# NVlabs/intrinsic3d

Measured on AMD Instinct MI355X. Metric: Gauss-Newton iterations/s at the finest SDF level, higher is better.
Workload: dtype f32

## Files before the change

### intrinsic3d_amd/csrc/device/kernels.hpp

```cpp
#pragma once
#include "common.hpp"
#include "p2p_device.hpp"

namespace i3d {

struct HashTable { unsigned long long* keys; int* vals; unsigned int mask; };
void launch_sort_keys(hipStream_t st, int N, const int* keys_xyz , unsigned long long* sort_keys, int* iota);
void launch_permute_grid(hipStream_t st, int N, const int* perm, const int* keys_xyz, const double* sdf, const double* sdf_ref,
                         const double* alb, const float* w, const uint8_t* rgb,
                         int* cx, int* cy, int* cz, int* rank, double* sdf0, double* x_sdf, double* x_alb, float* f_sdf, float* f_alb,
                         float* weight, uchar4* color);
void launch_hash_build(hipStream_t st, int N, const int* cx, const int* cy, const int* cz, HashTable t);
void launch_nbr_build(hipStream_t st, int N, const int* cx, const int* cy, const int* cz, HashTable t, int* nbr);
void launch_classify(hipStream_t st, GridView g, OptParams p, int* active_flag);
void launch_compact(hipStream_t st, int N, const int* active_flag, const int* active_scan, const uint8_t* flags, int* aidx, int* alist, uint8_t* aflags);
void launch_partition_blocks(hipStream_t st, GridView g, int A, int* alist, uint8_t* aflags, int* aidx);
void launch_group_rows(hipStream_t st, int A, const uint8_t* nrows, int* gmax);
void launch_anbr(hipStream_t st, int N, int A, int Acap, const int* alist, const int* nbr, const int* aidx, int* anbr);
void launch_scatter_sh(hipStream_t st, int N, const int* rank, const double* sh_visit , float* sh );
void launch_gather_visit(hipStream_t st, int N, const int* rank, const double* x_sdf, const double* x_alb, double* out_sdf, double* out_alb);
void launch_update_fields(hipStream_t st, int N, const int* rank, const double* sdf_ref, const double* alb, const uint8_t* rgb,
                          double* x_sdf, double* x_alb, float* f_sdf, float* f_alb, uchar4* color);

void launch_observe(hipStream_t st, GridView g, RowView r, OptParams p, const FrameConst* frames, const unsigned* cull_mask = nullptr, bool prefilter = false);
constexpr int CULL_BLOCK = 8, CULL_MAX_LEVELS = 12;
struct CullPyramid { int levels, cells; int bw[CULL_MAX_LEVELS], bh[CULL_MAX_LEVELS], off[CULL_MAX_LEVELS]; };
CullPyramid cull_pyramid(int w, int h);
void launch_depth_blocks(hipStream_t st, const FrameConst* frames, int K, int w, int h, float2* out);
void launch_group_cull(hipStream_t st, GridView g, RowView r, OptParams p, const FrameConst* frames, const float2* dblocks, float4* bounds, unsigned* mask);

void launch_build(hipStream_t st, GridView g, RowView r, OptParams p, const FrameConst* frames, bool with_jacobian, double* cost_out , double* scratch,
                  const double* cam9 = nullptr, const LmState* lm = nullptr);
void launch_weight_sums(hipStream_t st, RowView r, GridView g, bool with_cost, double* sums13 , double* scratch);

enum PassMode { PASS_GRAD = 0, PASS_JTJP = 1, PASS_COLNORM = 2 };
struct Seg2 { size_t off0, off1; int n; };
struct PassBuffers {
    float* C;
    float* treg;
    double* shared;
    double* blocks;
    float* part; int part_stride;
};
struct GradColBuffers {
    float* Cg; float* Cc;
    float* tregg; float* tregc;
    float* part; int part_stride;
    int col_off;
    double* cost_partials; double* cost_out;
};
int  launch_eg_gradcol(hipStream_t st, GridView g, RowView r, OptParams p, GradColBuffers b);
int  launch_eg_pass(hipStream_t st, PassMode mode, GridView g, RowView r, OptParams p, const float* u , PassBuffers b, const PcgState* state);
void launch_sum_rows(hipStream_t st, PassMode mode, int K, const float* part, int nrows, int stride, double* shared, double* blocks);
void launch_gather(hipStream_t st, PassMode mode, RowView r, PassBuffers b, float* out );
int  launch_gather_tail(hipStream_t st, RowView r, PassBuffers b, float* out, const float* S, const float* D2, const float* v, double* dot_partials ,
                        bool dot_atomic, const PcgState* state);
void launch_reduce_partials(hipStream_t st, const double* partials, int nblk, int ncomp, double* dst, const PcgState* state, bool assign = false);
void launch_shared_finalize(hipStream_t st, size_t tail_off, int K, OptParams p, const double* shared, float* out , bool tail, const float* S, const float* D2,
                            const float* v, double* dot_out, const PcgState* state);

void launch_fill(hipStream_t st, int n, float* x, float v);
void launch_fill_d(hipStream_t st, int n, double* x, double v);
void launch_int_to_double(hipStream_t st, const int* src, double* dst);
void launch_mul(hipStream_t st, int n, const float* a, const float* b, float* out);
void launch_scale_from_colnorm(hipStream_t st, int n, const float* c, const float* freemask, float* S, float* cm);
void launch_dot(hipStream_t st, int n, const float* a, const float* b, double* out , double* scratch);
void launch_count_above2(hipStream_t st, Seg2 sg, const float* a, const float* m, float tol, double* out, double* scratch);
void launch_count_above(hipStream_t st, int n, const float* a, const float* m, float tol, double* out, double* scratch);
void launch_dot2(hipStream_t st, Seg2 sg, const float* a, const float* b, double* out , double* scratch);
void launch_mul2(hipStream_t st, Seg2 sg, const float* a, const float* b, float* out);
void launch_freemask(hipStream_t st, RowView r, OptParams p, float* mask );

void launch_pcg_init(hipStream_t st, PcgState* state, int fixed_iterations, int max_iterations, const LmState* lm = nullptr);
int  launch_pcg_step(hipStream_t st, int mode, Seg2 sg, const float* p, const float* q, float* x, float* r, const float* b, const float* D2, const float* Minv,
                     float* z, const float* S_for_inline_q, double* partials , PcgState* state);
void launch_pcg_tail_x(hipStream_t st, size_t tail_off, int K, const float* p, float* x, const PcgState* state);
void launch_pcg_tail_a(hipStream_t st, int mode, size_t tail_off, int K, const float* Minv_blocks, const float* p, const float* q, float* x, float* r, const float* b,
                       const float* D2, float* z, const double* partials, int nblk, PcgState* state,
                       double* shared_zero, int nzero, int* host_flags, int seq,
                       const P2PDev& pd);
int  launch_pcg_direction(hipStream_t st, Seg2 sg, size_t tail_off, int ntail, const float* z, float* p, const float* S, float* u, const float* D2,
                          double* d2_partials , const PcgState* state);
void launch_pcg_tail_b(hipStream_t st, size_t tail_off, int K, OptParams p, double* shared, const double* pq_slice, const double* pq_partials, int nblk,
                       const double* pq_partials2, int nblk2, bool rowwise,
                       float* q, const float* S, const float* D2, const float* v, PcgState* state, const P2PDev& pd);
struct TilePlan {
    unsigned* lnbr;
    float* eaw_sym;
    int* halo_idx; int* halo_cnt;
    int* iota; int* ext_e; int* ext_pos;
    float* qh;
    int* ext_off;
    int* overflow;
    int T, hmax;
    int tile_first, ntiles_own;
    const int* ghost_tiles; int n_ghost;
    int det;
    const unsigned short* hp_off;
    const unsigned short* hp_src;
    int pull;
};
inline int tile_plan_pull_cap(int hmax) { return 4 * hmax; }
inline int tile_plan_hmax_of(int T) { return T == 1024 ? 2048 : 1536; }
inline int tile_plan_tiles_of(int A, int T) { return (A + T - 1) / T; }
size_t tile_plan_temp_bytes(size_t nslots);
hipError_t launch_tile_plan(hipStream_t st, RowView r, TilePlan t, int hmax_limit , void* temp, size_t temp_bytes);
void launch_eaw_sym(hipStream_t st, RowView r, TilePlan t, const int* cflag );
int  launch_eg_tile(hipStream_t st, RowView r, OptParams p, const float* u, TilePlan t, double* shared, float* qacc, double* pq_partials ,
                    const PcgState* state, float* cam_partials = nullptr, int cam_stride = 0);
void launch_ext_offsets(hipStream_t st, int n, const int* ext_e, int A, int* ext_off);
void eg_tile_launch_shape(const TilePlan& t, int K, int& blocks, int& tiles_per_block);

struct LadVec;
int  eg_tile_mr_max_systems(int K);
int  launch_eg_tile_mr(hipStream_t st, RowView r, OptParams p, TilePlan t, int nsys, const int* sys, const float* u0, float* qacc0, float* qh0, double* pq0 , float* cam0, int cam_stride,
                       const PcgState* st0 , const LadVec& lv);
int  launch_eg_tile_mr_pair(hipStream_t st, RowView r, OptParams p, TilePlan t, int na, int nb, const int* sys, const float* u0, float* qacc0, float* qh0, double* pq0 , float* cam0,
                            int cam_stride, const PcgState* st0, const LadVec& lv);

struct ShardArgs {
    P2PDev pd; RimLists rim; int seq;
    int n_slice_partials;
    int n_rim_wg;
    const float* zb; float* pb; float* ub; const float* cmb; int chunk;
};
struct LadVec {
    size_t vec;
    size_t qh;
    size_t cam;
    size_t part;
    size_t mblk;
    size_t tail;
    int sysid[LADDER_MAX];
};
struct Step3Args {
    int nq; int chunk4;
    const float4* p; const float4* qacc; float4* x; float4* r; const float4* b; float4* z;
    const float4* cm; const LmState* lm;
    const int* ext_off; const int* ext_pos; const float2* qh; int e0;
    const double* pq_partials; int n_pq; const double* d2_partials; int n_d2;
    int n_slice_wg;
    int K; int fix_poses, fix_intr, fix_dist;
    const float* cam_partials; int n_cam; int cam_stride; const float* Mblk;
    const float* tp; float* tx; float* tr; const float* tb; const float* tD2; float* tz; const float* tS;
    double* step_partials;
    PcgState* cur;
    int sharded; ShardArgs sh;
    int lad_sys;
    const double* redop; int redop_stride;
};
void launch_pcg_init3(hipStream_t st, PcgState* st2 , int fixed_iterations, int max_iterations, const LmState* lm = nullptr);
int  launch_pcg_dir3(hipStream_t st, bool init, Seg2 sg, size_t tail_off, int ntail, const float* z, float* p, const float* S, float* u, const float* D2, const float* cm, const LmState* lm,
                     const double* step_partials, int n_step, double* d2_partials, const PcgState* prev, PcgState* next, int* host_flags, int seq,
                     const ShardArgs* sa = nullptr);
void launch_rim_u(hipStream_t st, const ShardArgs& sa, const PcgState* state);
int  pcg_step3_slice_wgs(int n_entries, int cap = 0);
int  pcg_step3_tail_wgs(int K);
int  launch_pcg_step3(hipStream_t st, int mode , Step3Args a);
void launch_halo_fold(hipStream_t st, RowView r, TilePlan t, float* qacc, const PcgState* state);
void launch_pcg_init_lad(hipStream_t st, PcgState* st2_all , int B, int fixed_iterations, int max_iterations, const LmState* lm);
int  launch_pcg_dir3_lad(hipStream_t st, bool init, int nsys, Seg2 sg, size_t tail_off, int ntail, const float* z0, float* p0, const float* S, float* u0, const float* tD2_0, const float* cm, const LmState* lm,
                         const double* step_partials0, int n_step, double* d2_partials0, PcgState* st2_0, int prev_parity, int* host_flags0, int seq, const LadVec& lv,
                         int n_slice_partials = 0, const double* red4_0 = nullptr );
int  launch_pcg_step3_lad(hipStream_t st, int mode, int nsys, Step3Args a, const LadVec& lv);
void launch_lad_reduce_step(hipStream_t st, int nsys, const double* step_partials0, int n_slice, double* red4_0, const LadVec& lv);
void launch_lad_reduce_op(hipStream_t st, int nsys, const float* cam_partials0, int n_cam, int cam_stride, int NS, const double* pq_partials0, int n_pq, const double* d2_partials0, int n_d2,
                          double* redop0, int redop_stride, const LadVec& lv);

void launch_need_mask(hipStream_t st, RowView r, int slice, unsigned long long* need );
void launch_halo_items(hipStream_t st, int A, int slice, int me, const unsigned long long* need, unsigned long long* items, int* count , int cap);
void launch_tile_flags(hipStream_t st, int A, int T, const int* cflag, int* tileflag );
size_t halo_sort_temp_bytes(int cap);
hipError_t launch_halo_sort(hipStream_t st, void* temp, size_t temp_bytes, const unsigned long long* in, unsigned long long* out, int n);

void launch_candidate(hipStream_t st, GridView g, RowView r, int K, float sign, const float* step, const float* S, const double* x_shared, double* xc_sdf, double* xc_alb,
                      double* xc_shared, double* norms2 , const float* mask, double* scratch, const LmState* lm = nullptr);
void launch_accept(hipStream_t st, GridView g, RowView r, const double* xc_sdf, const double* xc_alb, const LmState* lm = nullptr);
void launch_set_double(hipStream_t st, double* dst, double v);
void launch_lm_init(hipStream_t st, LmState* lm, const double* cost, const double* ngrad, const double* nfree, double radius0, LmRecord* rec, int seq);
void launch_lm_begin(hipStream_t st, LmState* lm, int K, int fix_poses, int fix_intr, int fix_dist, const double* cdiag, const double* tri, float* Mblk,
                     const float* tc, const float* tS, float* tD2, float* tMinv, LmRecord* rec, int seq);
void launch_lm_diag_dev(hipStream_t st, int n, const float* c, const float* S, const LmState* lm, float* D2, float* Minv);
void launch_cand_frames(hipStream_t st, int K, const double* xc, const FrameConst* base, FrameConst* out, const LmState* lm);
void launch_lm_decide(hipStream_t st, LmState* lm, const PcgState* ps, const double* norms2, const double* cand_cost, int attempt, int lm_steps, LmRecord* rec, int seq,
                      int lad_next = -1 , int debug_invalid = 0);
void launch_lm_begin_lad(hipStream_t st, LmState* lm, int B, int K, int fix_poses, int fix_intr, int fix_dist, const double* cdiag, const double* tri, float* Mblk, size_t mblk_stride,
                         const float* tc, const float* tS, float* tD2, size_t tail_stride, LmRecord* rec, int seq);
void launch_mark_compute(hipStream_t st, RowView r, int* flag);
void launch_compact_list(hipStream_t st, int A, const int* flag, const int* scan, int* list);

}
```

### intrinsic3d_amd/csrc/device/pcg_fused.hip

```cpp
#include "kernels.hpp"
#include "reduce_device.hpp"
#include <cstring>

namespace i3d {

constexpr int PF_THREADS = 512;
constexpr int PF_MAX_WG = 512;
constexpr int PF_POSES_PER_WG = 10;

template <int NC>
static __device__ inline void reduce_partials_all(const double* __restrict__ P, int nblk, double (&tot)[NC], double* sm ,
                                                  const double* __restrict__ P2 = nullptr, int nblk2 = 0 ) {
    double v[NC];
#pragma unroll
    for (int k = 0; k < NC; ++k) v[k] = 0.0;
    for (int i = threadIdx.x; i < nblk; i += PF_THREADS) {
#pragma unroll
        for (int k = 0; k < NC; ++k) v[k] += P[(size_t)i * NC + k];
    }
    for (int i = threadIdx.x; i < nblk2; i += PF_THREADS) {
#pragma unroll
        for (int k = 0; k < NC; ++k) v[k] += P2[(size_t)i * NC + k];
    }
#pragma unroll
    for (int k = 0; k < NC; ++k) for (int o = 32; o > 0; o >>= 1) v[k] += __shfl_down(v[k], o, 64);
    if ((threadIdx.x & 63) == 0) {
#pragma unroll
        for (int k = 0; k < NC; ++k) sm[k * 8 + (threadIdx.x >> 6)] = v[k];
    }
    __syncthreads();
#pragma unroll
    for (int k = 0; k < NC; ++k) { double t = 0.0; for (int w = 0; w < PF_THREADS / 64; ++w) t += sm[k * 8 + w]; tot[k] = t; }
    __syncthreads();
}

__global__ void k_pcg_init3(PcgState* st2, int fixed_iterations, int max_iterations, const LmState* lm) {
    const bool over = lm && lm->done;
    for (int b = 0; b < 2; ++b) {
        PcgState* st = st2 + b;
        for (int k = 0; k < 4; ++k) st->acc[k] = 0.0;
        st->rho = 0.0; st->last_rho = 1.0; st->pq = 0.0; st->alpha = 0.0; st->beta = 0.0; st->xbr = 0.0; st->xr = 0.0; st->d2xx = 0.0;
        st->Q0 = 0.0; st->Q1 = 0.0; st->it = 0; st->done = (fixed_iterations == 0 || over) ? 1 : 0; st->fixed_iterations = fixed_iterations; st->max_iterations = max_iterations;
    }
}
void launch_pcg_init3(hipStream_t st, PcgState* st2, int fixed_iterations, int max_iterations, const LmState* lm) { k_pcg_init3<<<1, 1, 0, st>>>(st2, fixed_iterations, max_iterations, lm); }

static __device__ inline void lm_from_colnorm(float cm, float inv_radius, float& s, float& d2, float& minv) { s = lm_scale(cm); lm_diag(cm, s, inv_radius, d2, minv); }

template <int SH>
static __device__ __forceinline__ void pcg_dir3_body(int init, int n4, int seg4, size_t tail_rel, int ntail, const float* __restrict__ z, float* __restrict__ p,
                                                        const float* __restrict__ S, float* __restrict__ u, const float* __restrict__ tD2 ,
                                                        const float* __restrict__ cm, const float inv_radius, const double* __restrict__ step_partials, int n_step, double* __restrict__ d2_partials,
                                                        const PcgState* __restrict__ prev, PcgState* __restrict__ next, int* host_flags, int seq, const ShardArgs& sa,
                                                        const double* __restrict__ red4 = nullptr ) {
    __shared__ double sm[4 * 8];
    __shared__ double smx[SH == 1 ? 4 * P2P_MAX_RANKS : 1];
    auto publish = [&](int done) { if (host_flags) { __hip_atomic_store(&host_flags[2 * (seq & 1) + 1], done, __ATOMIC_RELAXED, __HIP_MEMORY_SCOPE_SYSTEM);
                                                     __hip_atomic_store(&host_flags[2 * (seq & 1)], seq, __ATOMIC_RELEASE, __HIP_MEMORY_SCOPE_SYSTEM); } };
    const int n_rim = SH == 1 ? sa.n_rim_wg : 0, n_main = SH ? (int)gridDim.x - n_rim - 1 : (int)gridDim.x;
    const int lid = SH == 1 ? ((int)blockIdx.x < n_rim ? n_main + 1 + (int)blockIdx.x : (int)blockIdx.x - n_rim) : (int)blockIdx.x;
    const bool rim_wg = SH == 1 && lid > n_main, tail_wg = SH ? lid == n_main : lid == n_main - 1;
    const bool writer = lid == 0 && threadIdx.x == 0;
    const float4* z4 = reinterpret_cast<const float4*>(z); float4* p4 = reinterpret_cast<float4*>(p);
    const float4* C4 = reinterpret_cast<const float4*>(cm); float4* u4 = reinterpret_cast<float4*>(u);
    if (prev->done) { if (writer) { *next = *prev; publish(prev->done); } return; }
    double tot[4];
    if (!SH) reduce_partials_all<4>(step_partials, n_step, tot, sm);
    else if (SH == 2) {
        reduce_partials_all<4>(step_partials + 4 * (size_t)sa.n_slice_partials, n_step - sa.n_slice_partials, tot, sm);
#pragma unroll
        for (int k = 0; k < 4; ++k) tot[k] += red4[k];
    } else {
        const unsigned e32 = p2p_pass_epoch(seq, P2P_X_DIR);
        if (rim_wg) {
            const RimLists& rl = sa.rim;
            for (int j = (lid - n_main - 1) * PF_THREADS + threadIdx.x; j < rl.n_send; j += n_rim * PF_THREADS) {
                const int e = rl.send_idx[j], k = rl.send_peer[j];
                p2p_put_rim(sa.pd, 0, e32, k, j - rl.send_off[k], sa.zb[e], sa.zb[(size_t)sa.chunk + e]);
            }
        }
        {   double loc[4];
            reduce_partials_all<4>(step_partials, sa.n_slice_partials, loc, sm);
            if (lid == 0 && threadIdx.x < 4) p2p_put_double_all(sa.pd, 0, e32, threadIdx.x, threadIdx.x == 0 ? loc[0] : threadIdx.x == 1 ? loc[1] : threadIdx.x == 2 ? loc[2] : loc[3]); }
        double tl[4];
        reduce_partials_all<4>(step_partials + 4 * (size_t)sa.n_slice_partials, n_step - sa.n_slice_partials, tl, sm);
        p2p_sum_all<4>(sa.pd, 0, e32, tot, smx);
#pragma unroll
        for (int k = 0; k < 4; ++k) tot[k] += tl[k];
    }
    int it = prev->it, done = 0; bool stop = false;
    double Q0 = prev->Q0, Q1 = prev->Q1, xbr = prev->xbr, xr = prev->xr, d2xx = prev->d2xx;
    if (!init) {
        xbr = tot[1]; xr = tot[2]; d2xx = tot[3];
        it = it + 1;
        Q1 = -tot[1];
        if (prev->fixed_iterations >= 0) { Q0 = Q1; if (it >= prev->fixed_iterations) { done = 1; stop = true; } }
        else {
            const double zeta = (double)it * (Q1 - Q0) / Q1;
            if (zeta < 0.1) { done = 1; stop = true; }
            else { Q0 = Q1; if (it >= prev->max_iterations) { done = 1; stop = true; } }
        }
    }
    double rho = prev->rho, last_rho = prev->last_rho, beta = prev->beta;
    if (!stop) {
        const double rho_new = tot[0];
        if (rho_new == 0.0 || isinf(rho_new) || isnan(rho_new)) { done = 2; stop = true; }
        else {
            if (it > 0) { const double bt = rho_new / prev->rho; if (bt == 0.0 || isinf(bt) || isnan(bt)) { done = 2; stop = true; } else beta = bt; }
            else beta = 0.0;
            if (!stop) { last_rho = prev->rho; rho = rho_new; }
        }
    }
    if (writer) {
        PcgState s = *prev;
        s.rho = rho; s.last_rho = last_rho; s.beta = beta; s.xbr = xbr; s.xr = xr; s.d2xx = d2xx; s.Q0 = Q0; s.Q1 = Q1; s.it = it; s.done = done; s.pq = 0.0;
        *next = s;
        publish(done);
    }
    if (stop) return;
    const float betaf = (float)beta; const bool first = it == 0;
    if (rim_wg) {
        const RimLists& rl = sa.rim; const unsigned e32 = p2p_pass_epoch(seq, P2P_X_DIR);
        for (int j = (lid - n_main - 1) * PF_THREADS + threadIdx.x; j < rl.n_recv; j += n_rim * PF_THREADS) {
            const int e = rl.recv_idx[j], k = rl.recv_peer[j];
            float zs, za; p2p_get_rim(sa.pd, 0, e32, k, j - rl.recv_off[k], zs, za);
            const size_t ea = (size_t)sa.chunk + e;
            const float ps = first ? zs : zs + betaf * sa.pb[e], pa = first ? za : za + betaf * sa.pb[ea];
            sa.pb[e] = ps; sa.pb[ea] = pa;
            sa.ub[e] = lm_scale(sa.cmb[e]) * ps; sa.ub[ea] = lm_scale(sa.cmb[ea]) * pa;
        }
        return;
    }
    double d2 = 0.0;
    if (!SH || !tail_wg) {
        for (int j = lid * PF_THREADS + threadIdx.x; j < 2 * n4; j += n_main * PF_THREADS) {
            const int i = j < n4 ? j : j - n4 + seg4;
            float4 pi = z4[i]; const float4 cv = C4[i];
            if (!first) { const float4 po = p4[i]; pi.x += betaf * po.x; pi.y += betaf * po.y; pi.z += betaf * po.z; pi.w += betaf * po.w; }
            p4[i] = pi;
            float4 sv, dd; float mi;
            lm_from_colnorm(cv.x, inv_radius, sv.x, dd.x, mi); lm_from_colnorm(cv.y, inv_radius, sv.y, dd.y, mi);
            lm_from_colnorm(cv.z, inv_radius, sv.z, dd.z, mi); lm_from_colnorm(cv.w, inv_radius, sv.w, dd.w, mi);
            u4[i] = make_float4(sv.x * pi.x, sv.y * pi.y, sv.z * pi.z, sv.w * pi.w);
            d2 += (double)dd.x * (double)pi.x * (double)pi.x + (double)dd.y * (double)pi.y * (double)pi.y + (double)dd.z * (double)pi.z * (double)pi.z + (double)dd.w * (double)pi.w * (double)pi.w;
        }
    }
    if (tail_wg) {
        for (int t = threadIdx.x; t < ntail; t += PF_THREADS) {
            const size_t i = tail_rel + t;
            const float pi = first ? z[i] : z[i] + betaf * p[i]; p[i] = pi; u[i] = S[i] * pi;
            d2 += (double)tD2[t] * (double)pi * (double)pi;
        }
    }
    { const double t = block_sum_d(d2); if (threadIdx.x == 0) d2_partials[lid] = t; }
}
template <int SH>
__global__ void __launch_bounds__(PF_THREADS, SH ? 4 : 1) k_pcg_dir3(int init, int n4, int seg4, size_t tail_rel, int ntail, const float* __restrict__ z, float* __restrict__ p,
                                                        const float* __restrict__ S, float* __restrict__ u, const float* __restrict__ D2 ,
                                                        const float* __restrict__ cm, const LmState* __restrict__ lm, const double* __restrict__ step_partials, int n_step, double* __restrict__ d2_partials,
                                                        const PcgState* __restrict__ prev, PcgState* __restrict__ next, int* host_flags, int seq, ShardArgs sa) {
    pcg_dir3_body<SH>(init, n4, seg4, tail_rel, ntail, z, p, S, u, D2 + tail_rel, cm, lm->inv_radius , step_partials, n_step, d2_partials, prev, next, host_flags, seq, sa);
}
template <bool COLL>
__global__ void __launch_bounds__(PF_THREADS, 1) k_pcg_dir3_lad(int init, int n4, int seg4, size_t tail_rel, int ntail, const float* __restrict__ z0, float* __restrict__ p0,
                                                        const float* __restrict__ S, float* __restrict__ u0, const float* __restrict__ tD2_0, const float* __restrict__ cm, const LmState* __restrict__ lm,
                                                        const double* __restrict__ step_partials0, int n_step, double* __restrict__ d2_partials0, PcgState* __restrict__ st2_0 , int prev_parity,
                                                        int* host_flags0, int seq, LadVec lv, int n_slice_partials, const double* __restrict__ red4_0) {
    const int j = lv.sysid[blockIdx.y];
    ShardArgs none; none.n_rim_wg = 0; none.n_slice_partials = n_slice_partials;
    const size_t vo = (size_t)j * lv.vec;
    pcg_dir3_body<COLL ? 2 : 0>(init, n4, seg4, tail_rel, ntail, z0 + vo, p0 + vo, S, u0 + vo, tD2_0 + (size_t)j * lv.tail, cm, lm->lad_inv_radius[j], step_partials0 + (size_t)j * lv.part, n_step,
                                d2_partials0 + (size_t)j * lv.part, st2_0 + 2 * j + prev_parity, st2_0 + 2 * j + (prev_parity ^ 1), host_flags0 + 4 * j, seq, none, COLL ? red4_0 + 4 * j : nullptr);
}

static int dir3_main_wgs(int n_entries, int cap) { int b = (n_entries / 2 + PF_THREADS - 1) / PF_THREADS; b = b < 1 ? 1 : b; return b > cap ? cap : b; }
int launch_pcg_dir3(hipStream_t st, bool init, Seg2 sg, size_t tail_off, int ntail, const float* z, float* p, const float* S, float* u, const float* D2, const float* cm, const LmState* lm,
                    const double* step_partials, int n_step, double* d2_partials, const PcgState* prev, PcgState* next, int* host_flags, int seq, const ShardArgs* sa) {
    const int n4 = sg.n >> 2, seg4 = (int)((sg.off1 - sg.off0) >> 2);
    const size_t o = sg.off0;
    if (!sa) {
        const int blocks = dir3_main_wgs(sg.n, PF_MAX_WG);
        ShardArgs none; std::memset(&none, 0, sizeof(none));
        k_pcg_dir3<0><<<blocks, PF_THREADS, 0, st>>>(init ? 1 : 0, n4, seg4, tail_off - o, ntail, z + o, p + o, S + o, u + o, D2 + o, cm + o, lm, step_partials, n_step, d2_partials, prev, next, host_flags, seq, none);
        return blocks;
    }
    const int cap = sa->pd.wg_cap > 0 ? sa->pd.wg_cap : PF_MAX_WG;
    const int n_main = dir3_main_wgs(sg.n, cap);
    k_pcg_dir3<1><<<sa->n_rim_wg + n_main + 1, PF_THREADS, 0, st>>>(init ? 1 : 0, n4, seg4, tail_off - o, ntail, z + o, p + o, S + o, u + o, D2 + o, cm + o, lm, step_partials, n_step, d2_partials, prev, next,
                                                                       host_flags, seq, *sa);
    return n_main;
}

int launch_pcg_dir3_lad(hipStream_t st, bool init, int nsys, Seg2 sg, size_t tail_off, int ntail, const float* z0, float* p0, const float* S, float* u0, const float* tD2_0, const float* cm, const LmState* lm,
                        const double* step_partials0, int n_step, double* d2_partials0, PcgState* st2_0, int prev_parity, int* host_flags0, int seq, const LadVec& lv,
                        int n_slice_partials, const double* red4_0) {
    const int n4 = sg.n >> 2, seg4 = (int)((sg.off1 - sg.off0) >> 2);
    const size_t o = sg.off0;
    const int blocks = dir3_main_wgs(sg.n, PF_MAX_WG);
    if (red4_0)
        k_pcg_dir3_lad<true><<<dim3(blocks + 1, nsys), PF_THREADS, 0, st>>>(init ? 1 : 0, n4, seg4, tail_off - o, ntail, z0 + o, p0 + o, S + o, u0 + o, tD2_0, cm + o, lm, step_partials0, n_step, d2_partials0,
                                                                            st2_0, prev_parity, host_flags0, seq, lv, n_slice_partials, red4_0);
    else
        k_pcg_dir3_lad<false><<<dim3(blocks, nsys), PF_THREADS, 0, st>>>(init ? 1 : 0, n4, seg4, tail_off - o, ntail, z0 + o, p0 + o, S + o, u0 + o, tD2_0, cm + o, lm, step_partials0, n_step, d2_partials0,
                                                                         st2_0, prev_parity, host_flags0, seq, lv, 0, nullptr);
    return blocks;
}

__global__ void __launch_bounds__(PF_THREADS) k_rim_u(ShardArgs sa, const PcgState* __restrict__ state) {
    if (state->done) return;
    const RimLists& rl = sa.rim; const unsigned e32 = p2p_pass_epoch(sa.seq, P2P_X_RESET_RIM);
    for (int j = blockIdx.x * PF_THREADS + threadIdx.x; j < rl.n_send; j += gridDim.x * PF_THREADS) {
        const int e = rl.send_idx[j], k = rl.send_peer[j];
        p2p_put_rim(sa.pd, 0, e32, k, j - rl.send_off[k], sa.ub[e], sa.ub[(size_t)sa.chunk + e]);
    }
    for (int j = blockIdx.x * PF_THREADS + threadIdx.x; j < rl.n_recv; j += gridDim.x * PF_THREADS) {
        const int e = rl.recv_idx[j], k = rl.recv_peer[j];
        float us, ua; p2p_get_rim(sa.pd, 0, e32, k, j - rl.recv_off[k], us, ua);
        sa.ub[e] = us; sa.ub[(size_t)sa.chunk + e] = ua;
    }
}
void launch_rim_u(hipStream_t st, const ShardArgs& sa, const PcgState* state) { if (sa.rim.n_send > 0 || sa.rim.n_recv > 0) k_rim_u<<<sa.n_rim_wg > 0 ? sa.n_rim_wg : 1, PF_THREADS, 0, st>>>(sa, state); }

enum { S3_INIT = 0, S3_NORMAL = 1, S3_XONLY = 2, S3_RESET = 3 };


struct S3Off { size_t v4, vo, qh2, part, cam, mblk, tail; int st, sys; };
struct S3In { float4 as, aa; int4 o; int o4; float4 x[2], p[2], b[2], cm[2], r[2]; };
template <int MODE> static __device__ inline void s3_load(const Step3Args& a, const S3Off& o, int q, S3In& v) {
    const float4* const qacc = a.qacc + o.v4; const float4* const x = a.x + o.v4; const float4* const p = a.p + o.v4; const float4* const r = a.r + o.v4;
    if (MODE == S3_NORMAL || MODE == S3_RESET) {
        v.as = qacc[q]; v.aa = qacc[q + a.chunk4];
        const int e = a.e0 + 4 * q;
        v.o = *reinterpret_cast<const int4*>(a.ext_off + e);
        v.o4 = a.ext_off[e + 4];
    }
#pragma unroll
    for (int seg = 0; seg < 2; ++seg) {
        const int i = q + seg * a.chunk4;
        v.cm[seg] = a.cm[i];
        if (MODE == S3_INIT) v.r[seg] = r[i];
        else {
            v.x[seg] = x[i];
            if (MODE != S3_RESET) v.p[seg] = p[i];
            if (MODE != S3_XONLY) { v.b[seg] = a.b[i]; if (MODE == S3_NORMAL) v.r[seg] = r[i]; }
        }
    }
}

template <int MODE, int SH>
static __device__ __forceinline__ void pcg_step3_body(const Step3Args& a, const S3Off& o) {
    __shared__ double sm[4 * 8];
    __shared__ double smx[SH == 1 ? P2P_MAX_RANKS : 1];
    __shared__ double camv[64];
    __shared__ double camred[8][64];
    __shared__ float rs[64];
    PcgState* const cur = a.cur + o.st;
    float4* const X = a.x + o.v4; float4* const R = a.r + o.v4; float4* const Z = a.z + o.v4;
    const double* const pq_partials = a.pq_partials + o.part; const double* const d2_partials = a.d2_partials + o.part; double* const step_partials = a.step_partials + o.part;
    const float2* const qh = a.qh + o.qh2; const float* const cam_partials = a.cam_partials + o.cam; const float* const Mblk = a.Mblk + o.mblk;
    const float* const tp = a.tp + o.vo; float* const tx = a.tx + o.vo; float* const tr = a.tr + o.vo; float* const tz = a.tz + o.vo; const float* const tD2 = a.tD2 + o.tail;
    const bool slice_wg = (int)blockIdx.x < a.n_slice_wg;
    const int q0 = blockIdx.x * PF_THREADS + threadIdx.x, qstride = a.n_slice_wg * PF_THREADS;
    S3In in;
    __shared__ int done_s;
    if (threadIdx.x == 0) done_s = cur->done;
    __syncthreads();
    if (done_s) return;
    const float inv_radius = o.sys >= 0 ? a.lm->lad_inv_radius[o.sys] : a.lm->inv_radius;
    float alpha = 0.0f;
    if (MODE == S3_NORMAL || MODE == S3_XONLY) {
        double t1[1];
        if (SH == 2) t1[0] = a.redop[(size_t)(o.sys < 0 ? 0 : o.sys) * a.redop_stride + 6 * a.K + 9] + d2_partials[a.n_d2];
        else reduce_partials_all<1>(pq_partials, a.n_pq, t1, sm, d2_partials, a.n_d2);
        if (SH == 1) {
            const unsigned e32 = p2p_pass_epoch(a.sh.seq, P2P_X_STEP);
            if (blockIdx.x == 0 && threadIdx.x == 0) p2p_put_double_all(a.sh.pd, 1, e32, 0, t1[0]);
            p2p_sum_all<1>(a.sh.pd, 1, e32, t1, smx);
            t1[0] += d2_partials[a.n_d2];
        }
        const double pq = t1[0];
        const double al = cur->rho / pq;
        const bool bad = !(pq > 0.0) || isinf(pq) || isinf(al);
        if (blockIdx.x == 0 && threadIdx.x == 0) { cur->pq = pq; if (bad) cur->done = 2; else cur->alpha = al; }
        if (bad) return;
        alpha = (float)al;
    }
    double s0 = 0.0, s1 = 0.0, s2 = 0.0, s3 = 0.0;
    if (slice_wg) {
        for (int q = q0; q < a.nq; q += qstride) {
            s3_load<MODE>(a, o, q, in);
            float accv[2][4];
            if (MODE == S3_NORMAL || MODE == S3_RESET) {
                const float4 as = in.as, aa = in.aa;
                accv[0][0] = as.x; accv[0][1] = as.y; accv[0][2] = as.z; accv[0][3] = as.w; accv[1][0] = aa.x; accv[1][1] = aa.y; accv[1][2] = aa.z; accv[1][3] = aa.w;
                const int ob[5] = {in.o.x, in.o.y, in.o.z, in.o.w, in.o4};
                for (int j0 = ob[0]; j0 < ob[4]; j0 += 8) {
                    int pos[8]; float2 hv[8];
#pragma unroll
                    for (int u = 0; u < 8; ++u) pos[u] = (j0 + u < ob[4]) ? a.ext_pos[j0 + u] : -1;
#pragma unroll
                    for (int u = 0; u < 8; ++u) hv[u] = pos[u] >= 0 ? qh[pos[u]] : make_float2(0.0f, 0.0f);
#pragma unroll
                    for (int u = 0; u < 8; ++u) {
                        const int j = j0 + u;
                        if (j < ob[4]) {
#pragma unroll
                            for (int k = 0; k < 4; ++k) { const bool mine = j >= ob[k] && j < ob[k + 1]; accv[0][k] += mine ? hv[u].x : 0.0f; accv[1][k] += mine ? hv[u].y : 0.0f; }
                        }
                    }
                }
            }
#pragma unroll
            for (int seg = 0; seg < 2; ++seg) {
                const int i = q + seg * a.chunk4;
                float xv[4], rv[4], svv[4], dv[4], mv[4];
                { const float4 cv = in.cm[seg]; lm_from_colnorm(cv.x, inv_radius, svv[0], dv[0], mv[0]); lm_from_colnorm(cv.y, inv_radius, svv[1], dv[1], mv[1]);
                  lm_from_colnorm(cv.z, inv_radius, svv[2], dv[2], mv[2]); lm_from_colnorm(cv.w, inv_radius, svv[3], dv[3], mv[3]); }
                if (MODE == S3_INIT) { const float4 t = in.r[seg]; rv[0] = t.x; rv[1] = t.y; rv[2] = t.z; rv[3] = t.w; }
                else {
                    const float4 xo = in.x[seg];
                    xv[0] = xo.x; xv[1] = xo.y; xv[2] = xo.z; xv[3] = xo.w;
                    float pv[4] = {0.0f, 0.0f, 0.0f, 0.0f};
                    if (MODE != S3_RESET) {
                        const float4 pp = in.p[seg]; pv[0] = pp.x; pv[1] = pp.y; pv[2] = pp.z; pv[3] = pp.w;
#pragma unroll
                        for (int k = 0; k < 4; ++k) xv[k] += alpha * pv[k];
                        X[i] = make_float4(xv[0], xv[1], xv[2], xv[3]);
                    }
                    if (MODE == S3_XONLY) continue;
                    const float4 bb = in.b[seg];
                    const float bv[4] = {bb.x, bb.y, bb.z, bb.w};
                    float qq[4];
#pragma unroll
                    for (int k = 0; k < 4; ++k) qq[k] = svv[k] * accv[seg][k] + dv[k] * (MODE == S3_NORMAL ? pv[k] : xv[k]);
                    if (MODE == S3_NORMAL) { const float4 ro = in.r[seg]; rv[0] = ro.x - alpha * qq[0]; rv[1] = ro.y - alpha * qq[1]; rv[2] = ro.z - alpha * qq[2]; rv[3] = ro.w - alpha * qq[3]; }
                    else { rv[0] = bv[0] - qq[0]; rv[1] = bv[1] - qq[1]; rv[2] = bv[2] - qq[2]; rv[3] = bv[3] - qq[3]; }
                    R[i] = make_float4(rv[0], rv[1], rv[2], rv[3]);
#pragma unroll
                    for (int k = 0; k < 4; ++k) { const double xd = xv[k]; s1 += xd * ((double)bv[k] + (double)rv[k]); s2 += xd * (double)rv[k]; s3 += (double)dv[k] * xd * xd; }
                }
                const float zv[4] = {mv[0] * rv[0], mv[1] * rv[1], mv[2] * rv[2], mv[3] * rv[3]};
                Z[i] = make_float4(zv[0], zv[1], zv[2], zv[3]);
#pragma unroll
                for (int k = 0; k < 4; ++k) s0 += (double)rv[k] * (double)zv[k];
            }
        }
    } else {
        const int K = a.K, tw = (int)blockIdx.x - a.n_slice_wg, n_pose_wg = (K + PF_POSES_PER_WG - 1) / PF_POSES_PER_WG;
        int col0, ncol;
        if (tw < n_pose_wg) { col0 = 6 * PF_POSES_PER_WG * tw; const int c1 = min(6 * K, col0 + 6 * PF_POSES_PER_WG); ncol = c1 - col0; }
        else { col0 = 6 * K; ncol = 9; }
        const int t = threadIdx.x;
        if (MODE == S3_NORMAL || MODE == S3_RESET) {
            const int g = t / 64, c = t % 64;
            double v = 0.0;
            if (SH != 2 && c < ncol) for (int w = g; w < a.n_cam; w += 8) v += (double)cam_partials[(size_t)w * a.cam_stride + col0 + c];
            camred[g][c] = v;
            __syncthreads();
            if (t < ncol) {
                double s = 0.0; for (int gg = 0; gg < 8; ++gg) s += camred[gg][t];
                if (SH == 2) s = a.redop[(size_t)(o.sys < 0 ? 0 : o.sys) * a.redop_stride + col0 + t];
                if (SH == 1) {
                    const unsigned e32 = p2p_pass_epoch(a.sh.seq, MODE == S3_RESET ? P2P_X_RESET_STEP : P2P_X_STEP);
                    p2p_put_double_all(a.sh.pd, 1, e32, 1 + col0 + t, s);
                    s = 0.0; for (int j = 0; j < a.sh.pd.L.world; ++j) s += p2p_get_double(a.sh.pd, 1, e32, j, 1 + col0 + t);
                }
                camv[t] = s;
            }
            __syncthreads();
        }
        if (t < ncol) {
            const int i = col0 + t;
            const bool fixed = i < 6 * K ? a.fix_poses : (i < 6 * K + 4 ? a.fix_intr : a.fix_dist);
            float ri;
            if (MODE == S3_INIT) ri = tr[i];
            else {
                float xi = tx[i];
                if (MODE != S3_RESET) { xi += alpha * tp[i]; tx[i] = xi; }
                if (MODE == S3_XONLY) ri = 0.0f;
                else {
                    const float vv = MODE == S3_NORMAL ? tp[i] : xi;
                    const float qi = a.tS[i] * (fixed ? 0.0f : (float)camv[t]) + tD2[i] * vv;
                    ri = MODE == S3_NORMAL ? tr[i] - alpha * qi : a.tb[i] - qi;
                    tr[i] = ri;
                    const double xd = xi; s1 += xd * ((double)a.tb[i] + (double)ri); s2 += xd * (double)ri; s3 += (double)tD2[i] * xd * xd;
                }
            }
            rs[t] = ri;
        }
        if (MODE == S3_XONLY) return;
        __syncthreads();
        if (t < ncol) {
            const int i = col0 + t;
            int base, n, row; const float* M;
            if (i < 6 * K) { const int f = i / 6; base = 6 * f; n = 6; row = i - base; M = Mblk + 36 * f; }
            else if (i < 6 * K + 4) { base = 6 * K; n = 4; row = i - base; M = Mblk + 36 * K; }
            else { base = 6 * K + 4; n = 5; row = i - base; M = Mblk + 36 * K + 16; }
            float s = 0.0f;
            for (int j = 0; j < n; ++j) s += M[row * n + j] * rs[base - col0 + j];
            tz[i] = s; s0 += (double)rs[t] * (double)s;
        }
    }
    if (MODE == S3_XONLY) return;
    block_partial_d(s0, step_partials, 4, 0); block_partial_d(s1, step_partials, 4, 1); block_partial_d(s2, step_partials, 4, 2); block_partial_d(s3, step_partials, 4, 3);
}
template <int MODE, int SH>
__global__ void __launch_bounds__(PF_THREADS) k_pcg_step3(Step3Args a) { const S3Off o{0, 0, 0, 0, 0, 0, 0, 0, -1}; pcg_step3_body<MODE, SH>(a, o); }
template <int MODE, bool COLL>
__global__ void __launch_bounds__(PF_THREADS) k_pcg_step3_lad(Step3Args a, LadVec lv) {
    const int j = lv.sysid[blockIdx.y];
    const S3Off o{((size_t)j * lv.vec) >> 2, (size_t)j * lv.vec, ((size_t)j * lv.qh) >> 1, (size_t)j * lv.part, (size_t)j * lv.cam, (size_t)j * lv.mblk, (size_t)j * lv.tail, 2 * j, j};
    pcg_step3_body<MODE, COLL ? 2 : 0>(a, o);
}

int pcg_step3_slice_wgs(int n_entries, int cap) { if (cap <= 0 || cap > PF_MAX_WG) cap = PF_MAX_WG; int b = (n_entries / 4 + PF_THREADS - 1) / PF_THREADS; return b < 1 ? 1 : (b > cap ? cap : b); }
int pcg_step3_tail_wgs(int K) { return (K + PF_POSES_PER_WG - 1) / PF_POSES_PER_WG + 1; }

int launch_pcg_step3(hipStream_t st, int mode, Step3Args a) {
    const int blocks = a.n_slice_wg + pcg_step3_tail_wgs(a.K);
#define I3D_S3(M) do { if (a.sharded) k_pcg_step3<M, 1><<<blocks, PF_THREADS, 0, st>>>(a); else k_pcg_step3<M, 0><<<blocks, PF_THREADS, 0, st>>>(a); } while (0)
    switch (mode) {
        case S3_INIT:   I3D_S3(S3_INIT); break;
        case S3_NORMAL: I3D_S3(S3_NORMAL); break;
        case S3_XONLY:  I3D_S3(S3_XONLY); break;
        default:        I3D_S3(S3_RESET); break;
    }
#undef I3D_S3
    return mode == S3_XONLY ? 0 : blocks;
}

int launch_pcg_step3_lad(hipStream_t st, int mode, int nsys, Step3Args a, const LadVec& lv) {
    const int blocks = a.n_slice_wg + pcg_step3_tail_wgs(a.K);
    const dim3 grid(blocks, nsys);
#define I3D_S3L(M) do { if (a.redop) k_pcg_step3_lad<M, true><<<grid, PF_THREADS, 0, st>>>(a, lv); else k_pcg_step3_lad<M, false><<<grid, PF_THREADS, 0, st>>>(a, lv); } while (0)
    switch (mode) {
        case S3_INIT:   I3D_S3L(S3_INIT); break;
        case S3_NORMAL: I3D_S3L(S3_NORMAL); break;
        case S3_XONLY:  I3D_S3L(S3_XONLY); break;
        default:        I3D_S3L(S3_RESET); break;
    }
#undef I3D_S3L
    return mode == S3_XONLY ? 0 : blocks;
}

__global__ void __launch_bounds__(PF_THREADS) k_lad_reduce_step(const double* __restrict__ step_partials0, int n_slice, double* __restrict__ red4_0, LadVec lv) {
    __shared__ double sm[4 * 8];
    const int j = lv.sysid[blockIdx.x];
    double tot[4];
    reduce_partials_all<4>(step_partials0 + (size_t)j * lv.part, n_slice, tot, sm);
    if (threadIdx.x < 4) red4_0[4 * j + threadIdx.x] = threadIdx.x == 0 ? tot[0] : threadIdx.x == 1 ? tot[1] : threadIdx.x == 2 ? tot[2] : tot[3];
}
void launch_lad_reduce_step(hipStream_t st, int nsys, const double* step_partials0, int n_slice, double* red4_0, const LadVec& lv) {
    k_lad_reduce_step<<<nsys, PF_THREADS, 0, st>>>(step_partials0, n_slice, red4_0, lv);
}
__global__ void __launch_bounds__(PF_THREADS) k_lad_reduce_op(const float* __restrict__ cam_partials0, int n_cam, int cam_stride, int NS, const double* __restrict__ pq_partials0, int n_pq,
                                                              const double* __restrict__ d2_partials0, int n_d2, double* __restrict__ redop0, int redop_stride, LadVec lv) {
    __shared__ double sm[8];
    __shared__ double camred[8][64];
    const int j = lv.sysid[blockIdx.y];
    double* const out = redop0 + (size_t)j * redop_stride;
    const int ncw = (NS + 63) / 64;
    if ((int)blockIdx.x < ncw) {
        const int t = threadIdx.x, g = t / 64, c = t % 64, col = (int)blockIdx.x * 64 + c;
        const float* cp = cam_partials0 + (size_t)j * lv.cam;
        double v = 0.0;
        if (col < NS) for (int w = g; w < n_cam; w += 8) v += (double)cp[(size_t)w * cam_stride + col];
        camred[g][c] = v;
        __syncthreads();
        if (t < 64 && col < NS) { double s = 0.0; for (int gg = 0; gg < 8; ++gg) s += camred[gg][t]; out[col] = s; }
    } else {
        double t1[1];
        reduce_partials_all<1>(pq_partials0 + (size_t)j * lv.part, n_pq, t1, sm, d2_partials0 + (size_t)j * lv.part, n_d2);
        if (threadIdx.x == 0) out[NS] = t1[0];
    }
}
void launch_lad_reduce_op(hipStream_t st, int nsys, const float* cam_partials0, int n_cam, int cam_stride, int NS, const double* pq_partials0, int n_pq, const double* d2_partials0, int n_d2,
                          double* redop0, int redop_stride, const LadVec& lv) {
    k_lad_reduce_op<<<dim3((NS + 63) / 64 + 1, nsys), PF_THREADS, 0, st>>>(cam_partials0, n_cam, cam_stride, NS, pq_partials0, n_pq, d2_partials0, n_d2, redop0, redop_stride, lv);
}

__global__ void k_pcg_init_lad(PcgState* st2_all, int B, int fixed_iterations, int max_iterations, const LmState* lm) {
    const int j = threadIdx.x;
    if (j >= B) return;
    const bool over = lm->done != 0 || lm->lad_radius[j] < 1e-32;
    for (int b = 0; b < 2; ++b) {
        PcgState* st = st2_all + 2 * j + b;
        for (int k = 0; k < 4; ++k) st->acc[k] = 0.0;
        st->rho = 0.0; st->last_rho = 1.0; st->pq = 0.0; st->alpha = 0.0; st->beta = 0.0; st->xbr = 0.0; st->xr = 0.0; st->d2xx = 0.0;
        st->Q0 = 0.0; st->Q1 = 0.0; st->it = 0; st->done = (fixed_iterations == 0 || over) ? 1 : 0; st->fixed_iterations = fixed_iterations; st->max_iterations = max_iterations;
    }
}
void launch_pcg_init_lad(hipStream_t st, PcgState* st2_all, int B, int fixed_iterations, int max_iterations, const LmState* lm) { k_pcg_init_lad<<<1, LADDER_MAX, 0, st>>>(st2_all, B, fixed_iterations, max_iterations, lm); }

__global__ void k_ext_offsets(int n, const int* __restrict__ ext_e, int A, int* __restrict__ ext_off) {
    const int e = blockIdx.x * blockDim.x + threadIdx.x;
    if (e > A) return;
    int lo = 0, hi = n;
    while (lo < hi) { const int mid = (lo + hi) >> 1; if (ext_e[mid] < e) lo = mid + 1; else hi = mid; }
    ext_off[e] = lo;
}
void launch_ext_offsets(hipStream_t st, int n, const int* ext_e, int A, int* ext_off) { k_ext_offsets<<<(A + 1 + 255) / 256, 256, 0, st>>>(n, ext_e, A, ext_off); }

}
```

### intrinsic3d_amd/csrc/host/context.hpp

```cpp
#pragma once
#include <functional>
#include <string>
#include <vector>
#include <cstring>
#include <cmath>
#include "../device/kernels.hpp"
#include "../device/render_kernels.hpp"
#include "../device/track_kernels.hpp"
#include "../device/query_kernels.hpp"
#include "../device/register_kernels.hpp"
#include "../device/track_sdf_kernels.hpp"
#include "comm.hpp"
#include "../../../include/intrinsic3d_hip.h"

namespace i3d {

template <class T>
struct DevBuf {
    T* p = nullptr; size_t n = 0;
    DevBuf() = default;
    DevBuf(const DevBuf&) = delete; DevBuf& operator=(const DevBuf&) = delete;
    DevBuf(DevBuf&& o) noexcept : p(o.p), n(o.n) { o.p = nullptr; o.n = 0; }
    DevBuf& operator=(DevBuf&& o) noexcept { if (this != &o) { release(); p = o.p; n = o.n; o.p = nullptr; o.n = 0; } return *this; }
    ~DevBuf() { release(); }
    void release() { if (p) (void)hipFree(p); p = nullptr; n = 0; }
    hipError_t alloc(size_t count) {
        if (count <= n && p) return hipSuccess;
        release();
        if (count == 0) return hipSuccess;
        hipError_t e = hipMalloc((void**)&p, count * sizeof(T));
        if (e == hipSuccess) n = count;
        return e;
    }
};

struct PinnedBuf {
    unsigned char* p = nullptr; size_t n = 0;
    PinnedBuf() = default;
    PinnedBuf(const PinnedBuf&) = delete; PinnedBuf& operator=(const PinnedBuf&) = delete;
    ~PinnedBuf() { release(); }
    void release() { if (p) (void)hipHostFree(p); p = nullptr; n = 0; }
    hipError_t alloc(size_t bytes) {
        if (bytes <= n) return hipSuccess;
        release();
        hipError_t e = hipHostMalloc((void**)&p, bytes);
        if (e == hipSuccess) n = bytes;
        return e;
    }
};

inline double rms_of(double sq, double n) { return n > 0.0 ? std::sqrt(sq / n) : 0.0; }

struct TrackBuffers {
    DevBuf<float> pyr, vn, model, lum; DevBuf<double> slab; DevBuf<TrackState> state; DevBuf<RenderStatsDev> rstats;
};

struct TrackModel {
    std::function<int(int code, const std::string& msg)> fail;
    std::function<int(const i3d_track_desc& d, const double*& intr, const double*& dist)> ready;
    std::function<void(const RenderCam& cam, const RenderPlanes& out, RenderStatsDev* stats)> cast;
    std::function<int()> intensity_ready;
};

struct TrackRgbd {
    const float* luminance; double geometric_weight, photo_weight; float max_photo_residual;
    int64_t photo_samples = 0; double photo_rms_initial = 0.0, photo_rms_final = 0.0;
};

int track_frame_run(hipStream_t st, TrackBuffers& b, const TrackModel& m, const char* what, const i3d_track_desc* d, int32_t w, int32_t h, const float* depth,
                    double* pose6_io, i3d_track_stats* stats, TrackRgbd* rgbd = nullptr);
int track_sums_run(hipStream_t st, TrackBuffers& b, const TrackModel& m, const char* what, const i3d_track_desc* d, int32_t w, int32_t h, const float* depth,
                   int32_t level, const double* pose_ref6, const double* pose_cur6, double* sums, int64_t* inliers, TrackRgbd* rgbd = nullptr);

struct QueryModel {
    std::function<int(int code, const std::string& msg)> fail;
    std::function<int()> ready;
    std::function<void(const QueryParams& p, const double* points, const QueryOut& out, QueryRow* rows, QueryRow* total)> launch;
    double voxel_size;
};
int query_run(hipStream_t st, DevBuf<unsigned char>& scratch, const QueryModel& m, const char* what, const i3d_query_desc* d, int64_t n, const double* points,
              double* sdf, float* normal, float* albedo, double* foot, double* distance, uint8_t* status, i3d_query_stats* stats);

void rot_to_aa(const double R[9], double aa[3]);
struct Pose { double R[9], t[3]; };
Pose pose_from_vec6(const double* p6);
void vec6_from_pose(const Pose& P, double* p6);

struct RegisterModel {
    std::function<int(int code, const std::string& msg)> fail;
    std::function<int()> ready;
    std::function<void(const RegisterParams& p, const double* points, const TrackState* state, int check_done, double* slab)> launch;
    double voxel_size;
    int row_cap = REGISTER_MAX_ROWS;
};
int register_run(hipStream_t st, DevBuf<unsigned char>& scratch, const RegisterModel& m, const char* what, const i3d_register_desc* d, int64_t n, const double* points,
                 double* pose6_io, i3d_register_stats* stats, const double* debug_pivot3 = nullptr, double* debug_sums29 = nullptr, int64_t* debug_valid = nullptr);

struct RegisterLoop {
    double* slab; TrackState* state;
    long long n; int per_lane;
    std::function<void(const double* R0, const double* t0)> mean;
    std::function<void(const RegisterParams& p, int check_done)> pass;
    int iterations; double stop_rotation, stop_translation, max_distance;
    const double* debug_pivot3 = nullptr; double* debug_sums29 = nullptr; int64_t* debug_valid = nullptr;
};
int register_loop(hipStream_t st, const std::function<int(int code, const std::string& msg)>& fail, const RegisterLoop& lp, double* pose6_io, i3d_register_stats& out);

void pivot_of(const double* sums, const double* R0, const double* t0, double* c);
void start_state(TrackState& hs, const double* R0, const double* t0, const double* c);

struct TrackSdfModel {
    std::function<int(int code, const std::string& msg)> fail;
    std::function<int(const i3d_track_sdf_desc& d, const double*& intr, const double*& dist)> ready;
    std::function<int()> intensity_ready;
    std::function<int(const double*& vol)> intensity;
    std::function<void(const TrackSdfParams& p, const TrackSdfPhoto* ph, const TrackSdfBatch& b, int check_done)> launch;
    double voxel_size;
    int row_cap = REGISTER_MAX_ROWS;
};
struct TrackSdfBuffers { DevBuf<unsigned char> scratch; PinnedBuf staging; };
struct TrackSdfRgbd {
    double geometric_weight, photo_weight; float max_photo_residual;
    i3d_track_sdf_rgbd_stats* stats = nullptr;
};
struct TrackSdfFrames {
    int32_t num, w, h;
    const float* host_depth; const float* const* dev_depth;
    const float* host_lum; const float* const* dev_lum;
};
struct TrackSdfDebug { const double* pivot3; double* sums; int64_t* valid; int64_t* usable; int64_t* photo_samples; };
int track_sdf_chunks(hipStream_t st, TrackSdfBuffers& buf, const TrackSdfModel& m, const i3d_track_sdf_desc* d, const double* intr, const double* dist,
                     const TrackSdfFrames& fr, double* poses6_io, i3d_track_sdf_stats* stats, const TrackSdfRgbd* rgbd = nullptr, int max_chunk = 0,
                     const TrackSdfDebug* debug = nullptr);
int track_sdf_run(hipStream_t st, TrackSdfBuffers& buf, const TrackSdfModel& m, const char* what, const i3d_track_sdf_desc* d, int32_t w, int32_t h,
                  const float* depth, double* pose6_io, i3d_track_sdf_stats* stats, const TrackSdfRgbd* rgbd = nullptr, const float* luminance = nullptr,
                  const TrackSdfDebug* debug = nullptr);

struct SolverSwitches {
    int  deterministic = -1;
    int  ladder = LADDER_MAX;
    bool ladder_mr = true, ladder_mr1 = false, ladder_pair = true; int ladder_group = 3;
    bool egt_mr1 = false;
    int  egt_tile = 0;
    int  hmax_limit = 0, hmax_limit_1024 = 0;
    bool halo_pull = false, no_tile = false, gradcol = true, cost0 = true;
    int  no_cull = 0;
    int  debug_invalid_attempt = -1;
    int  sh_slab = 0;
};

struct OperatorPlan {
    bool deterministic = false;
    int  ladder_max = 1;
    bool mr1_serial = false;
    bool ladder_lists = false;
    bool halo_pull = false;
    int  tile_T = 0;
    bool tile_ok = false;
    bool pull_lists() const { return halo_pull || ladder_lists; }
};

struct ShardState {
    int chunk = 1, own0 = 0, own1 = 0, nC = 0, slice = 0, n_ghost_tiles = 0;
    DevBuf<int> clist, cflag, cscan;
    HaloPlan halo; DevBuf<unsigned long long> need_mask, halo_items, halo_sorted;
    DevBuf<int> halo_count, halo_send_idx, halo_recv_idx, halo_send_peer, halo_recv_peer, halo_offs, tile_flag, ghost_tiles;
    DevBuf<float> halo_send_buf, halo_recv_buf; DevBuf<unsigned char> halo_temp;
};

struct LadderState {
    int hint = 0, hint_prev = 0;
    LadVec strides{};
    DevBuf<float> vec;
    DevBuf<float> qh, cam, mblk, tail;
    DevBuf<double> part;
    DevBuf<double> red;
    DevBuf<PcgState> st;
    long long batches = 0, streams = 0, system_passes = 0, resyncs = 0, wasted = 0;
    long long pass_live[7] = {0, 0, 0, 0, 0, 0, 0}, paired = 0;
};

struct Timing {
    bool on = false;
    unsigned mask = ~0u;
    double ms[I3D_K_COUNT] = {0};
    long long launches[I3D_K_COUNT] = {0};
    std::vector<float> each[I3D_K_COUNT];
    struct Pending { hipEvent_t a, b; int cat; };
    std::vector<Pending> pending;
    std::vector<hipEvent_t> pool;
};

}

struct i3d_context {
    int device = 0;
    hipStream_t stream = nullptr;
    std::string err;

    int N = 0; float voxel_size = 0, truncation = 0;
    i3d::DevBuf<int> cx, cy, cz, rank, nbr, aidx, alist, aflag, ascan;
    i3d::DevBuf<double> sdf0, x_sdf, x_alb, xc_sdf, xc_alb;
    i3d::DevBuf<float> f_sdf, f_alb, weight, sh;
    i3d::DevBuf<uchar4> color;
    i3d::DevBuf<uint8_t> flags;
    i3d::DevBuf<unsigned char> scan_tmp; size_t scan_tmp_bytes = 0;
    i3d::DevBuf<unsigned long long> hkeys; i3d::DevBuf<int> hvals; unsigned int hmask = 0;
    bool have_grid = false, have_sh = false;
    i3d::DevBuf<unsigned> render_bits; i3d::DevBuf<int> render_bounds; int render_lo[3] = {0, 0, 0}, render_dim[3] = {0, 0, 0}; bool render_bricks_ok = false;
    i3d::DevBuf<float> render_planes; i3d::DevBuf<i3d::RenderStatsDev> render_stats;
    i3d::TrackBuffers track;
    i3d::DevBuf<unsigned char> query_scratch;
    i3d::DevBuf<unsigned char> register_scratch; int register_row_cap = i3d::REGISTER_MAX_ROWS;
    i3d::TrackSdfBuffers track_sdf; int track_batch_frames = 0;
    i3d::DevBuf<double> track_sdf_intensity;
    std::vector<unsigned long long> sv_keys; std::vector<double> sv_sh; float sv_size = 0.0f; bool have_subvolumes = false;

    int K = 0, levels = 0;
    std::vector<int> fw, fh;
    std::vector<i3d::DevBuf<float>> lum, depth;
    std::vector<i3d::DevBuf<uint8_t>> bgr;
    i3d::DevBuf<i3d::FrameConst> d_frames, d_frames_cand;
    bool have_frames = false;

    double intr[4] = {0, 0, 0, 0}, dist[5] = {0, 0, 0, 0, 0};
    std::vector<double> poses;
    bool have_camera = false;

    int Acap = 0, slots = 0, A = 0; long long n_active = 0;
    i3d::Comm* comm = nullptr; i3d::ShardState shard;
    bool sharded() const { return comm && (comm->world > 1 || comm->force); }
    i3d::DevBuf<int> obs_frame, anbr; i3d::DevBuf<float> obs_w, ea_w, C, treg;
    i3d::DevBuf<float4> rows; i3d::DevBuf<float2> row_wr;
    i3d::DevBuf<uint8_t> aflags, nrows, regflags, ea_free; i3d::DevBuf<int> gmax;
    i3d::DevBuf<float2> cull_blocks; i3d::DevBuf<float4> cull_bounds; i3d::DevBuf<unsigned> cull_mask; int cull_level = -1; bool cull_on = false;
    double cost_at_build = 0.0;
    i3d::DevBuf<float> C2, treg2, gc_part;
    i3d::DevBuf<float> aux_part;
    i3d::DevBuf<unsigned> tp_lnbr; i3d::DevBuf<int> tp_halo_idx, tp_halo_cnt, tp_iota, tp_ext_e, tp_ext_pos, tp_ext_off, tp_overflow; i3d::DevBuf<float> tp_qh, tp_eaw, cam_part;
    i3d::DevBuf<unsigned char> tp_temp;
    i3d::DevBuf<unsigned short> tp_hp_off, tp_hp_src;
    i3d::SolverSwitches sw;
    i3d::OperatorPlan op;
    i3d::LadderState ladder;
    double t_add_end = 0.0;
    int plan_T() const { return op.tile_T > 0 ? op.tile_T : (sw.egt_tile == 512 ? 512 : 1024); }
    int plan_hmax_limit() const { return plan_T() == 512 ? sw.hmax_limit : sw.hmax_limit_1024; }
    i3d::TilePlan tile_plan() const {
        const int T = plan_T();
        const bool sh = sharded();
        const int t0 = sh ? shard.own0 / T : 0, t1 = sh ? (shard.own1 + T - 1) / T : i3d::tile_plan_tiles_of(A, T);
        return i3d::TilePlan{tp_lnbr.p, tp_eaw.p, tp_halo_idx.p, tp_halo_cnt.p, tp_iota.p, tp_ext_e.p, tp_ext_pos.p, tp_qh.p, tp_ext_off.p, tp_overflow.p, T, i3d::tile_plan_hmax_of(T), t0, t1 > t0 ? t1 - t0 : 0,
                             shard.ghost_tiles.p, sh ? shard.n_ghost_tiles : 0, op.deterministic ? 1 : 0, op.pull_lists() ? tp_hp_off.p : nullptr, op.pull_lists() ? tp_hp_src.p : nullptr, op.halo_pull ? 1 : 0};
    }

    i3d::DevBuf<float> v_mask, v_c, v_S, v_cm, v_D2, v_Minv, v_b, v_x, v_r, v_p, v_z, v_q, v_u, v_acc, v_tmp, v_qacc;
    i3d::DevBuf<float> Minv_blocks;
    i3d::DevBuf<double> d_shared, d_blocks, d_scal, d_xshared, d_xcshared;
    i3d::DevBuf<i3d::PcgState> d_pcg, d_pcg2; i3d::DevBuf<double> d_partials;
    int* h_flags = nullptr; int* d_flags = nullptr; int pcg_seq = 1024;
    i3d::DevBuf<i3d::LmState> d_lm; i3d::LmRecord* h_lmrec = nullptr; i3d::LmRecord* d_lmrec = nullptr; int lm_seq = 1;
    i3d::DevBuf<double> d_cam_c, d_cam_H;
    hipEvent_t ev_asm[2] = {nullptr, nullptr};
    long long n_syncs = 0;
    double* h_pinned = nullptr; size_t h_pinned_n = 0;

    i3d::OptParams last_params; bool assembled = false;
    long long last_sizes[6] = {0, 0, 0, 0, 0, 0};
    i3d::Timing timing;

    i3d::GridView grid_view() const;
    i3d::RowView row_view() const;
};

namespace i3d {

int ctx_fail(i3d_context* c, int code, const std::string& msg);
int ctx_hip(i3d_context* c, hipError_t e, const char* what);
int ctx_launch_check(i3d_context* c);
#define CTX_HIP(c, expr) do { hipError_t _e = (expr); if (_e != hipSuccess) return i3d::ctx_hip((c), _e, #expr); } while (0)
void build_frame_consts(const i3d_context* c, int level, const double* poses, std::vector<FrameConst>& out);
int ensure_pinned(i3d_context* c, size_t n);
bool timing_begin(i3d_context* c, int cat);
void timing_end(i3d_context* c);
void timing_flush(i3d_context* c);
struct TimedScope { i3d_context* c; bool active; TimedScope(i3d_context* c_, int cat) : c(c_), active(timing_begin(c_, cat)) {} ~TimedScope() { if (active) timing_end(c); } };

struct GridStaging { DevBuf<int> kxyz; DevBuf<double> sdf, sdf_ref, alb; DevBuf<float> w; DevBuf<uint8_t> rgb; };
int set_grid_device(i3d_context* c, int N, float voxel_size, float truncation, GridStaging& st);

int render_ensure_bricks(i3d_context* c);
RenderGrid render_grid(const i3d_context* c, bool refined);
inline RenderGrid field_grid(const i3d_context* c, bool refined) {
    return RenderGrid{HashTable{c->hkeys.p, c->hvals.p, c->hmask}, c->nbr.p, c->N, c->weight.p, refined ? c->x_sdf.p : c->sdf0.p, c->x_alb.p, c->sh.p,
                      (double)c->voxel_size, nullptr, {0, 0, 0}, {0, 0, 0}};
}
RenderCam render_cam(const PinholeCam& k, const double* pose6, float min_depth, float max_depth);

int recompute_colors(i3d_context* c, float occlusion_distance, int num_observations);
int clear_outside_thin_shell(i3d_context* c, double thres_shell, int64_t* new_count);
int upsample_grid(i3d_context* c, int64_t* new_count);

void read_switches(i3d_context* c);
int assemble(i3d_context* c, const i3d_optimizer_config& cfg, int iteration, OptParams& p, i3d_iteration_stats* st);
int optimize(i3d_context* c, const i3d_optimizer_config& cfg, i3d_iteration_stats* stats);
int normal_eq_debug(i3d_context* c, double* gradient, double* jtj_diag, double* cost);
int jtj_apply_debug(i3d_context* c, const double* x, double* y);
int work_list_debug(i3d_context* c, int32_t* visit_index, int64_t capacity, int64_t* count);

int estimate_sh(i3d_context* c, float subvolume_size, double lambda_reg, double thres_shell, int* num_subvolumes, double* sh,
                int32_t* sub_index, int cap, i3d_sh_stats* stats);

}
```

### intrinsic3d_amd/csrc/host/pcg.cpp

```cpp
#include "solver_internal.hpp"
#include <algorithm>

namespace i3d {

int run_pass(i3d_context* c, PassMode mode, const OptParams& p, const float* u, float* out ) {
    hipStream_t s = c->stream; GridView g = c->grid_view(); RowView r = c->row_view(); const Layout L = layout_of(c);
    const int stride = (int)aux_part_stride(c->K);
    PassBuffers b{c->C.p, c->treg.p, c->d_shared.p, c->d_blocks.p, c->aux_part.p, stride};
    CTX_HIP(c, hipMemsetAsync(c->d_shared.p, 0, sizeof(double) * ((size_t)L.NS + 1), s));
    if (mode == PASS_COLNORM) CTX_HIP(c, hipMemsetAsync(c->d_blocks.p, 0, sizeof(double) * (21 * (size_t)c->K + 25), s));
    if (mode == PASS_JTJP && c->op.tile_ok && !c->sharded()) {
        const int NSP = (L.NS + 3) & ~3; int rows = 0;
        { TimedScope t(c, I3D_K_EG_PASS); rows = launch_eg_tile(s, r, p, u, c->tile_plan(), nullptr, out, nullptr, nullptr, c->cam_part.p, NSP); }
        { TimedScope t(c, I3D_K_GATHER); launch_halo_fold(s, r, c->tile_plan(), out, nullptr); }
        { TimedScope t(c, I3D_K_VECTOR); launch_mul(s, 2 * c->shard.chunk, c->v_mask.p, out, out);
          if (rows > 0) launch_sum_rows(s, PASS_JTJP, c->K, c->cam_part.p, rows, NSP, c->d_shared.p, c->d_blocks.p); }
    } else {
        int rows = 0;
        { TimedScope t(c, mode == PASS_JTJP ? I3D_K_EG_PASS : I3D_K_EG_AUX); rows = launch_eg_pass(s, mode, g, r, p, u, b, nullptr);
          if (rows > AUX_PART_ROWS) return ctx_fail(c, I3D_ERR_CAPACITY, "run_pass: more workgroups than rows of the camera partial buffer");
          if (rows > 0) launch_sum_rows(s, mode, c->K, c->aux_part.p, rows, stride, c->d_shared.p, c->d_blocks.p); }
        { TimedScope t(c, I3D_K_GATHER); launch_gather(s, mode, r, b, out); }
    }
    { int rc = allreduce(c, c->d_shared.p, (size_t)L.NS); if (rc) return rc; }
    if (mode == PASS_COLNORM) { int rc = allreduce(c, c->d_blocks.p, 21 * (size_t)c->K + 25); if (rc) return rc; }
    { TimedScope t(c, I3D_K_VECTOR); launch_shared_finalize(s, L.tail_off, c->K, p, c->d_shared.p, out, false, nullptr, nullptr, nullptr, nullptr, nullptr); }
    return I3D_OK;
}

int run_gradcol(i3d_context* c, const OptParams& p, const std::function<int()>& between) {
    hipStream_t s = c->stream; GridView g = c->grid_view(); RowView r = c->row_view(); const Layout L = layout_of(c);
    const int stride = (int)gc_part_stride(c->K), col_off = (int)gc_col_off(c->K);
    GradColBuffers gb{c->C.p, c->C2.p, c->treg.p, c->treg2.p, c->gc_part.p, stride, col_off, c->d_partials.p, c->d_scal.p + 16};
    CTX_HIP(c, hipMemsetAsync(c->d_scal.p + 16, 0, sizeof(double), s));
    CTX_HIP(c, hipMemsetAsync(c->d_shared.p, 0, sizeof(double) * ((size_t)L.NS + 1), s));
    CTX_HIP(c, hipMemsetAsync(c->d_blocks.p, 0, sizeof(double) * (21 * (size_t)c->K + 25), s));
    int rows = 0;
    { TimedScope t(c, I3D_K_EG_AUX); rows = launch_eg_gradcol(s, g, r, p, gb);
      if (rows > GC_PART_ROWS) return ctx_fail(c, I3D_ERR_CAPACITY, "run_gradcol: more workgroups than rows of the camera partial buffer");
      if (rows > 0) launch_sum_rows(s, PASS_COLNORM, c->K, c->gc_part.p + col_off, rows, stride, c->d_shared.p, c->d_blocks.p); }
    { PassBuffers b{c->C2.p, c->treg2.p, c->d_shared.p, c->d_blocks.p, nullptr, 0};
      TimedScope t(c, I3D_K_GATHER); launch_gather(s, PASS_COLNORM, r, b, c->v_c.p); }
    { TimedScope t(c, I3D_K_VECTOR); launch_shared_finalize(s, L.tail_off, c->K, p, c->d_shared.p, c->v_c.p, false, nullptr, nullptr, nullptr, nullptr, nullptr); }
    { int rc = between(); if (rc) return rc; }
    CTX_HIP(c, hipMemsetAsync(c->d_shared.p, 0, sizeof(double) * ((size_t)L.NS + 1), s));
    { TimedScope t(c, I3D_K_EG_AUX); if (rows > 0) launch_sum_rows(s, PASS_GRAD, c->K, c->gc_part.p, rows, stride, c->d_shared.p, c->d_blocks.p); }
    { PassBuffers b{c->C.p, c->treg.p, c->d_shared.p, c->d_blocks.p, nullptr, 0};
      TimedScope t(c, I3D_K_GATHER); launch_gather(s, PASS_GRAD, r, b, c->v_acc.p); }
    { TimedScope t(c, I3D_K_VECTOR); launch_shared_finalize(s, L.tail_off, c->K, p, c->d_shared.p, c->v_acc.p, false, nullptr, nullptr, nullptr, nullptr, nullptr); }
    return I3D_OK;
}

int dot_dev(i3d_context* c, const float* a, const float* b, double* slot) {
    const Layout L = layout_of(c);
    CTX_HIP(c, hipMemsetAsync(slot, 0, sizeof(double), c->stream));
    { TimedScope t(c, I3D_K_VECTOR); launch_dot2(c->stream, L.own, a, b, slot, c->d_partials.p); }
    { int rc = allreduce(c, slot, 1); if (rc) return rc; }
    { TimedScope t(c, I3D_K_VECTOR); launch_dot(c->stream, L.NS, a + L.tail_off, b + L.tail_off, slot, c->d_partials.p); }
    return I3D_OK;
}

int count_above_dev(i3d_context* c, const float* a, const float* m, float tol, double* slot) {
    const Layout L = layout_of(c);
    CTX_HIP(c, hipMemsetAsync(slot, 0, sizeof(double), c->stream));
    { TimedScope t(c, I3D_K_VECTOR); launch_count_above2(c->stream, L.own, a, m, tol, slot, c->d_partials.p); }
    { int rc = allreduce(c, slot, 1); if (rc) return rc; }
    { TimedScope t(c, I3D_K_VECTOR); launch_count_above(c->stream, L.NS, a + L.tail_off, m + L.tail_off, tol, slot, c->d_partials.p); }
    return I3D_OK;
}

int eval_cost_launch(i3d_context* c, const OptParams& p, bool candidate, const FrameConst* frames, const double* cam9, const LmState* lm) {
    GridView g = c->grid_view();
    if (candidate) { g.x_sdf = c->xc_sdf.p; g.x_alb = c->xc_alb.p; }
    { TimedScope t(c, I3D_K_COST); launch_build(c->stream, g, c->row_view(), p, frames, false, c->d_scal.p + 16, c->d_partials.p, cam9, lm); }
    return allreduce(c, c->d_scal.p + 16, 1);
}

constexpr int PCG_MAX_ITERATIONS = 500;
constexpr int PCG_MAX_PASSES = 520;
constexpr int PCG_RESET_PERIOD = 10;
constexpr int PCG_SEQ_STRIDE = 1024;

constexpr int PART_STEP = 4 * 2048, PART_PQ = 2048, PART_D2 = 2048;
struct Partials { double *step, *pq, *d2; };
static Partials partials_at(double* base) { return Partials{base, base + PART_STEP, base + PART_STEP + PART_PQ}; }

static int wait_pass(i3d_context* c, const int* ring, int want, const char* stalled, bool* done) {
    const double t_wait = now_s();
    while (__atomic_load_n(&ring[0], __ATOMIC_ACQUIRE) != want) {
        if (now_s() - t_wait > 30.0) { CTX_HIP(c, sync_stream(c)); if (__atomic_load_n(&ring[0], __ATOMIC_ACQUIRE) != want) return ctx_fail(c, I3D_ERR_HIP, stalled); }
    }
    *done = __atomic_load_n(&ring[1], __ATOMIC_ACQUIRE) != 0;
    return I3D_OK;
}
static int previous_pass_done(i3d_context* c, int it, int seq, bool* done) {
    if (it < 2) return I3D_OK;
    return wait_pass(c, c->h_flags + 2 * ((seq - 1) & 1), seq - 1, "pcg_solve: the device stopped publishing its state", done);
}

static int begin_passes(const i3d_context* c) { return c->pcg_seq; }
static void end_passes(i3d_context* c, int seq0) { c->pcg_seq = seq0 + PCG_SEQ_STRIDE; }

static void launch_u_from_x(i3d_context* c, const Layout& L, const float* x, float* u) {
    launch_mul2(c->stream, L.own, c->v_S.p, x, u); launch_mul(c->stream, L.NS, c->v_S.p + L.tail_off, x + L.tail_off, u + L.tail_off);
}

int pcg_solve(i3d_context* c, const SolveRoute& route, const i3d_optimizer_config& cfg, const OptParams& p, const PcgState** final_state) {
    hipStream_t s = c->stream;
    const Layout L = layout_of(c);
    const int K = c->K;
    const bool sh = c->sharded();
    GridView g = c->grid_view(); RowView r = c->row_view();
    PassBuffers pb{c->C.p, c->treg.p, c->d_shared.p, c->d_blocks.p, c->aux_part.p, (int)aux_part_stride(c->K)};
    PcgState* st = c->d_pcg.p;
    double* pq_slot = c->d_shared.p + L.NS;
    const size_t to = L.tail_off; const Seg2 own = L.own;
    { TimedScope t(c, I3D_K_VECTOR); launch_fill(s, (int)L.NP, c->v_x.p, 0.0f); launch_pcg_init(s, st, cfg.pcg_fixed_iterations, PCG_MAX_ITERATIONS, c->d_lm.p); }
    CTX_HIP(c, hipMemcpyAsync(c->v_r.p, c->v_b.p, sizeof(float) * L.NP, hipMemcpyDeviceToDevice, s));
    const Partials part = partials_at(c->d_partials.p);
    int n_pq = 0, n_step = 0, n_d2 = 0;
    const bool dev_reduce = route.exchange == Exchange::InKernelReduce;
    const P2PDev& pd = route.reduce_dev;
    auto rows_apply = [&](const float* v, float* out, bool with_dot, bool zero_first) -> int {
        if (zero_first) CTX_HIP(c, hipMemsetAsync(c->d_shared.p, 0, sizeof(double) * ((size_t)L.NS + 1), s));
        if (sh) {
            { int rc = push_halo(c, c->v_u.p); if (rc) return rc; }
            { TimedScope t(c, I3D_K_EG_PASS);
              n_pq = launch_eg_tile(s, r, p, c->v_u.p, c->tile_plan(), c->d_shared.p, c->v_qacc.p, with_dot ? part.pq : nullptr, st); }
            { TimedScope t(c, I3D_K_GATHER); launch_halo_fold(s, r, c->tile_plan(), c->v_qacc.p, st); }
            if (!with_dot) n_pq = 0;
            if (dev_reduce && with_dot) return I3D_OK;
            if (with_dot) { TimedScope t(c, I3D_K_VECTOR); launch_reduce_partials(s, part.pq, n_pq, 1, pq_slot, st); launch_reduce_partials(s, part.d2, n_d2, 1, pq_slot, st); }
            n_pq = 0;
            return allreduce(c, c->d_shared.p, (size_t)L.NS + 1);
        }
        { TimedScope t(c, I3D_K_EG_PASS); launch_eg_pass(s, PASS_JTJP, g, r, p, c->v_u.p, pb, st); }
        { TimedScope t(c, I3D_K_GATHER); n_pq = launch_gather_tail(s, r, pb, out, c->v_S.p, c->v_D2.p, v, with_dot ? part.pq : nullptr, false, st); }
        if (!with_dot) n_pq = 0;
        return I3D_OK;
    };
    auto fold_step = [&]() { if (sh && !dev_reduce) { launch_reduce_partials(s, part.step, n_step, 4, st->acc, st); n_step = 0; } };
    const float* const Sq = sh ? c->v_S.p : nullptr;
    { TimedScope t(c, I3D_K_VECTOR);
      n_step = launch_pcg_step(s, 0 , own, c->v_p.p, c->v_q.p, c->v_x.p, c->v_r.p, c->v_b.p, c->v_D2.p, c->v_Minv.p, c->v_z.p, nullptr, part.step, st);
      fold_step(); }
    int tail_mode = 0;
    const int seq0 = begin_passes(c);
    for (int it = 1;; ++it) {
        if (sh && !dev_reduce) { int rc = allreduce(c, st->acc, 4); if (rc) return rc; }
        if (dev_reduce) { c->comm->count_reduce(4); c->comm->count_reduce((size_t)L.NS + 1); }
        { TimedScope t(c, I3D_K_VECTOR);
          launch_pcg_tail_a(s, tail_mode, to, K, c->Minv_blocks.p, c->v_p.p, tail_mode == 3 ? c->v_tmp.p : c->v_q.p, c->v_x.p, c->v_r.p, c->v_b.p, c->v_D2.p, c->v_z.p,
                            part.step, n_step, st, c->d_shared.p, L.NS + 1, c->d_flags, seq0 + it, pd); }
        { TimedScope t(c, I3D_K_VECTOR);
          n_d2 = launch_pcg_direction(s, own, to, L.NS, c->v_z.p, c->v_p.p, c->v_S.p, c->v_u.p, c->v_D2.p, sh ? part.d2 : nullptr, st); }
        { int rc = rows_apply(c->v_p.p, c->v_q.p, true, false); if (rc) return rc; }
        { TimedScope t(c, I3D_K_VECTOR); launch_pcg_tail_b(s, to, K, p, c->d_shared.p, pq_slot, part.pq, n_pq, part.d2, dev_reduce ? n_d2 : 0, sh,
                                                           c->v_q.p, c->v_S.p, c->v_D2.p, c->v_p.p, st, pd); }
        if (it % PCG_RESET_PERIOD != 0) {
            TimedScope t(c, I3D_K_VECTOR);
            n_step = launch_pcg_step(s, 1, own, c->v_p.p, sh ? c->v_qacc.p : c->v_q.p, c->v_x.p, c->v_r.p, c->v_b.p, c->v_D2.p, c->v_Minv.p, c->v_z.p, Sq, part.step, st);
            fold_step();
            tail_mode = 1;
        } else {
            { TimedScope t(c, I3D_K_VECTOR);
              launch_pcg_step(s, 2, own, c->v_p.p, c->v_q.p, c->v_x.p, c->v_r.p, c->v_b.p, c->v_D2.p, c->v_Minv.p, c->v_z.p, nullptr, part.step, st);
              launch_pcg_tail_x(s, to, K, c->v_p.p, c->v_x.p, st);
              launch_u_from_x(c, L, c->v_x.p, c->v_u.p); }
            { int rc = rows_apply(c->v_x.p, c->v_tmp.p, false, true); if (rc) return rc; }
            { TimedScope t(c, I3D_K_VECTOR);
              launch_shared_finalize(s, to, K, p, c->d_shared.p, c->v_tmp.p, true, c->v_S.p, c->v_D2.p, c->v_x.p, nullptr, st);
              n_step = launch_pcg_step(s, 3, own, c->v_p.p, sh ? c->v_qacc.p : c->v_tmp.p, c->v_x.p, c->v_r.p, c->v_b.p, c->v_D2.p, c->v_Minv.p, c->v_z.p, Sq, part.step, st);
              fold_step(); }
            tail_mode = 3;
        }
        bool done = false;
        { const int rc = previous_pass_done(c, it, seq0 + it, &done); if (rc) return rc; }
        if (done || it > PCG_MAX_PASSES) break;
    }
    end_passes(c, seq0);
    *final_state = st;
    return I3D_OK;
}

static Step3Args step3_args(const i3d_context* c, const Layout& L, const OptParams& p, const TilePlan& tp, float* x, float* r, float* pv, float* z, const float* q, const float* qh,
                            const Partials& part, const float* cam, const float* Mblk, const float* tD2, int wg_cap) {
    const Seg2 own = L.own; const size_t to = L.tail_off;
    Step3Args a; std::memset(&a, 0, sizeof(a));
    auto c4 = [&](const float* v) { return reinterpret_cast<const float4*>(v + own.off0); };
    auto m4 = [&](float* v) { return reinterpret_cast<float4*>(v + own.off0); };
    a.nq = own.n >> 2; a.chunk4 = (int)((own.off1 - own.off0) >> 2);
    a.p = c4(pv); a.qacc = c4(q); a.x = m4(x); a.r = m4(r); a.b = c4(c->v_b.p); a.z = m4(z); a.cm = c4(c->v_cm.p); a.lm = c->d_lm.p;
    a.ext_off = tp.ext_off; a.ext_pos = tp.ext_pos; a.qh = reinterpret_cast<const float2*>(qh); a.e0 = (int)own.off0;
    a.pq_partials = part.pq; a.d2_partials = part.d2; a.n_pq = 0; a.n_d2 = 0;
    a.n_slice_wg = pcg_step3_slice_wgs(own.n, wg_cap);
    a.K = c->K; a.fix_poses = p.fix_poses; a.fix_intr = p.fix_intr; a.fix_dist = p.fix_dist;
    a.cam_partials = cam; a.n_cam = 0; a.cam_stride = (L.NS + 3) & ~3; a.Mblk = Mblk;
    a.tp = pv + to; a.tx = x + to; a.tr = r + to; a.tb = c->v_b.p + to; a.tD2 = tD2; a.tz = z + to; a.tS = c->v_S.p + to;
    a.step_partials = part.step;
    return a;
}

int pcg_solve_fused(i3d_context* c, const SolveRoute& route, const i3d_optimizer_config& cfg, const OptParams& p, const PcgState** final_state) {
    hipStream_t s = c->stream;
    const Layout L = layout_of(c);
    const size_t to = L.tail_off; const Seg2 own = L.own;
    RowView r = c->row_view(); TilePlan tp = c->tile_plan();
    const bool sh = route.exchange == Exchange::InKernel;
    ShardArgs sa; std::memset(&sa, 0, sizeof(sa));
    if (sh) {
        if (!c->comm->fused_exchange(&sa.pd) || L.NS + 2 > sa.pd.L.red_cap) return ctx_fail(c, I3D_ERR_STATE, "pcg_solve_fused: the in-kernel exchanges are not available");
        const ShardState& sd = c->shard; const HaloPlan& h = sd.halo;
        sa.rim = RimLists{h.n_send, h.n_recv, sd.halo_send_idx.p, sd.halo_send_peer.p, sd.halo_recv_idx.p, sd.halo_recv_peer.p, sd.halo_offs.p, sd.halo_offs.p + P2P_MAX_RANKS};
        sa.n_rim_wg = (h.n_send + h.n_recv) > 0 ? std::max(1, std::min(4, (std::max(h.n_send, h.n_recv) + 1023) / 1024)) : 1;
        sa.zb = c->v_z.p; sa.pb = c->v_p.p; sa.ub = c->v_u.p; sa.cmb = c->v_cm.p; sa.chunk = sd.chunk;
    }
    const int wg_cap = sh ? sa.pd.wg_cap : 0;
    PcgState* const st2 = c->d_pcg2.p;
    const int NSP = (L.NS + 3) & ~3;
    const Partials part = partials_at(c->d_partials.p);
    { TimedScope t(c, I3D_K_VECTOR); launch_fill(s, (int)L.NP, c->v_x.p, 0.0f); launch_pcg_init3(s, st2, cfg.pcg_fixed_iterations, PCG_MAX_ITERATIONS, c->d_lm.p); }
    CTX_HIP(c, hipMemcpyAsync(c->v_r.p, c->v_b.p, sizeof(float) * L.NP, hipMemcpyDeviceToDevice, s));
    Step3Args a = step3_args(c, L, p, tp, c->v_x.p, c->v_r.p, c->v_p.p, c->v_z.p, c->v_qacc.p, tp.qh, part, c->cam_part.p, c->Minv_blocks.p, c->v_D2.p + to, wg_cap);
    a.sharded = sh ? 1 : 0; a.lad_sys = -1;
    int n_step = 0;
    { TimedScope t(c, I3D_K_VECTOR); a.cur = st2; n_step = launch_pcg_step3(s, 0 , a); }
    const bool mr1 = c->op.mr1_serial && !sh && route.multi_system;
    auto op = [&](double* pq, const PcgState* cur) -> int {
        if (mr1) { const int sys0[3] = {0, 0, 0}; LadVec z; std::memset(&z, 0, sizeof(z));
                   return launch_eg_tile_mr(s, r, p, tp, 1, sys0, c->v_u.p, c->v_qacc.p, tp.qh, pq, c->cam_part.p, NSP, cur, z); }
        return launch_eg_tile(s, r, p, c->v_u.p, tp, nullptr, c->v_qacc.p, pq, cur, c->cam_part.p, NSP);
    };
    const int seq0 = begin_passes(c);
    int it = 1;
    for (;; ++it) {
        PcgState* const prev = st2 + ((it + 1) & 1); PcgState* const cur = st2 + (it & 1);
        sa.seq = seq0 + it; sa.n_slice_partials = a.n_slice_wg; a.sh = sa;
        { TimedScope t(c, I3D_K_VECTOR);
          a.n_d2 = launch_pcg_dir3(s, it == 1, own, to, L.NS, c->v_z.p, c->v_p.p, c->v_S.p, c->v_u.p, c->v_D2.p, c->v_cm.p, c->d_lm.p, part.step, n_step, part.d2, prev, cur, c->d_flags, seq0 + it,
                                   sh ? &sa : nullptr); }
        if (sh) { c->comm->count_reduce(4); c->comm->count_halo(c->shard.halo.n_send); c->comm->count_reduce((size_t)L.NS + 1); }
        { TimedScope t(c, I3D_K_EG_PASS); a.n_pq = op(part.pq, cur); a.n_cam = a.n_pq; }
        a.cur = cur;
        if (it % PCG_RESET_PERIOD != 0) { TimedScope t(c, I3D_K_VECTOR); n_step = launch_pcg_step3(s, 1, a); }
        else {
            { TimedScope t(c, I3D_K_VECTOR); launch_pcg_step3(s, 2, a); launch_u_from_x(c, L, c->v_x.p, c->v_u.p); }
            if (sh) { TimedScope t(c, I3D_K_COMM); launch_rim_u(s, sa, cur); c->comm->count_halo(c->shard.halo.n_send); }
            { TimedScope t(c, I3D_K_EG_PASS); a.n_cam = op(nullptr, cur); }
            { TimedScope t(c, I3D_K_VECTOR); n_step = launch_pcg_step3(s, 3, a); }
        }
        bool done = false;
        { const int rc = previous_pass_done(c, it, seq0 + it, &done); if (rc) return rc; }
        if (done || it > PCG_MAX_PASSES) break;
    }
    end_passes(c, seq0);
    *final_state = st2 + (it & 1);
    { const int lrc = ctx_launch_check(c); if (lrc) return lrc; }
    return I3D_OK;
}

static size_t lad_redop_stride(int NS) { return ((size_t)NS + 1 + 3) & ~(size_t)3; }
int alloc_ladder(i3d_context* c) {
    const Layout L = layout_of(c);
    const int nsys = c->op.ladder_max;
    LadderState& ld = c->ladder; LadVec& lv = ld.strides;
    const size_t vec = ((size_t)L.NP + 65535) & ~(size_t)65535;
    const size_t qh = 2 * (size_t)tile_plan_tiles_of((int)std::min((size_t)c->Acap, ((size_t)c->shard.chunk + 65535) & ~(size_t)65535), 512) * (size_t)tile_plan_hmax_of(512);
    const size_t cam = (size_t)2048 * (((size_t)L.NS + 3) & ~(size_t)3);
    lv.vec = vec; lv.qh = qh; lv.cam = cam; lv.part = PART_STEP + PART_PQ + PART_D2; lv.mblk = ((size_t)36 * c->K + 41 + 3) & ~(size_t)3; lv.tail = ((size_t)L.NS + 3) & ~(size_t)3;
    const bool fresh = ld.vec.n < (size_t)6 * nsys * vec || !ld.vec.p;
    bool ok = ld.vec.alloc((size_t)6 * nsys * vec) == hipSuccess;
    if (ok && fresh) ok = hipMemsetAsync(ld.vec.p, 0, sizeof(float) * ld.vec.n, c->stream) == hipSuccess;
    ok = ok && ld.qh.alloc((size_t)nsys * qh) == hipSuccess && ld.cam.alloc((size_t)nsys * cam) == hipSuccess && ld.part.alloc((size_t)nsys * lv.part) == hipSuccess
            && ld.mblk.alloc((size_t)nsys * lv.mblk) == hipSuccess && ld.tail.alloc((size_t)nsys * lv.tail) == hipSuccess && ld.st.alloc((size_t)2 * LADDER_MAX) == hipSuccess;
    if (ok && c->sharded()) {
        const size_t n = (size_t)LADDER_MAX * (4 + lad_redop_stride(L.NS));
        const bool fresh_r = ld.red.n < n || !ld.red.p;
        ok = ld.red.alloc(n) == hipSuccess;
        if (ok && fresh_r) ok = hipMemsetAsync(ld.red.p, 0, sizeof(double) * ld.red.n, c->stream) == hipSuccess;
    }
    if (!ok) {
        (void)hipGetLastError();
        ld.vec.release(); ld.qh.release(); ld.cam.release(); ld.part.release();
        std::fprintf(stderr, "[i3d] the slabs of the damping ladder (%d systems x %.1f MB) do not fit the device: this outer iteration runs the serial trust-region loop\n", nsys,
                     (double)(6 * vec + qh + cam) * 4.0 / 1e6);
        return 1;
    }
    return I3D_OK;
}

int pcg_solve_ladder(i3d_context* c, const SolveRoute& route, const i3d_optimizer_config& cfg, const OptParams& p, int B, const PcgState** finals) {
    hipStream_t s = c->stream;
    const Layout L = layout_of(c);
    const int K = c->K; const size_t to = L.tail_off; const Seg2 own = L.own;
    RowView r = c->row_view(); TilePlan tp = c->tile_plan();
    LadderState& ld = c->ladder; LadVec lv = ld.strides;
    float* const X0 = lad_vecp(c, LV_X); float* const R0 = lad_vecp(c, LV_R); float* const P0 = lad_vecp(c, LV_P); float* const Z0 = lad_vecp(c, LV_Z);
    float* const U0 = lad_vecp(c, LV_U); float* const Q0 = lad_vecp(c, LV_Q);
    PcgState* const st2 = ld.st.p;
    const int NSP = (L.NS + 3) & ~3;
    const Partials part0 = partials_at(ld.part.p);
    const bool use_mr = c->sw.ladder_mr;
    const bool mr1 = c->sw.ladder_mr1;
    const int mr_cap = std::min(c->sw.ladder_group, eg_tile_mr_max_systems(K));
    const bool pair = c->sw.ladder_pair;
    const bool mr_ok = use_mr && mr_cap >= 1 && route.multi_system;
    const bool sh = route.exchange == Exchange::Transport;
    double* const red4 = sh ? ld.red.p : nullptr;
    const int rstride = (int)lad_redop_stride(L.NS);
    double* const redop = sh ? ld.red.p + (size_t)LADDER_MAX * 4 : nullptr;
    { TimedScope t(c, I3D_K_VECTOR);
      for (int j = 0; j < B; ++j) { CTX_HIP(c, hipMemsetAsync(X0 + (size_t)j * lv.vec, 0, sizeof(float) * L.NP, s));
                                    CTX_HIP(c, hipMemcpyAsync(R0 + (size_t)j * lv.vec, c->v_b.p, sizeof(float) * L.NP, hipMemcpyDeviceToDevice, s)); }
      launch_pcg_init_lad(s, st2, B, cfg.pcg_fixed_iterations, PCG_MAX_ITERATIONS, c->d_lm.p); }
    Step3Args a = step3_args(c, L, p, tp, X0, R0, P0, Z0, Q0, ld.qh.p, part0, ld.cam.p, ld.mblk.p, ld.tail.p, 0);
    a.sharded = 0; a.lad_sys = 0; a.redop = redop; a.redop_stride = rstride;
    std::vector<int> live(B); for (int j = 0; j < B; ++j) live[j] = j;
    auto set_slots = [&]() { for (int q = 0; q < LADDER_MAX; ++q) lv.sysid[q] = live[q < (int)live.size() ? q : (int)live.size() - 1]; };
    auto rows_apply = [&](int parity, bool with_dot) -> int {
        int n = 0; const int nl = (int)live.size();
        if (sh) { TimedScope t(c, I3D_K_COMM);
                  if (c->comm->push_halo_multi(U0, lv.vec, live.data(), nl, c->shard.halo, s)) return -1; }
        if (mr_ok && (nl > 1 || mr1 || sh)) {
            const int groups = (nl + mr_cap - 1) / mr_cap;
            int at = 0;
            if (groups == 2 && pair && !sh && nl - (nl + 1) / 2 >= 2) {
                const int na = (nl + 1) / 2;
                TimedScope t(c, na == 2 ? I3D_K_EG_MR2 : I3D_K_EG_MR3);
                n = launch_eg_tile_mr_pair(s, r, p, tp, na, nl - na, live.data(), U0, Q0, ld.qh.p, with_dot ? part0.pq : nullptr, ld.cam.p, NSP, st2 + parity, lv);
                if (n > 0) { at = nl; ++ld.streams; ++ld.paired; }
            }
            for (int g = 0; g < groups && at < nl; ++g) {
                const int ng = (nl - at + (groups - g) - 1) / (groups - g);
                TimedScope t(c, ng == 1 ? I3D_K_EG_PASS : (ng == 2 ? I3D_K_EG_MR2 : I3D_K_EG_MR3));
                n = launch_eg_tile_mr(s, r, p, tp, ng, live.data() + at, U0, Q0, ld.qh.p, with_dot ? part0.pq : nullptr, ld.cam.p, NSP, st2 + parity, lv);
                if (n <= 0) return -1;
                at += ng; ++ld.streams;
            }
        } else {
            for (int j : live) {
                TilePlan tj = tp; tj.qh = ld.qh.p + (size_t)j * lv.qh;
                TimedScope t(c, I3D_K_EG_PASS);
                n = launch_eg_tile(s, r, p, U0 + (size_t)j * lv.vec, tj, nullptr, Q0 + (size_t)j * lv.vec, with_dot ? part0.pq + (size_t)j * lv.part : nullptr, st2 + 2 * j + parity,
                                   ld.cam.p + (size_t)j * lv.cam, NSP);
                ++ld.streams;
            }
        }
        ld.system_passes += nl; ++ld.pass_live[nl < 6 ? nl : 6];
        if (sh) {
            { TimedScope t(c, I3D_K_VECTOR); launch_lad_reduce_op(s, nl, ld.cam.p, n, NSP, L.NS, part0.pq, with_dot ? n : 0, part0.d2, with_dot ? a.n_d2 : 0, redop, rstride, lv); }
            if (allreduce(c, redop, (size_t)LADDER_MAX * rstride)) return -1;
        }
        return n;
    };
    auto step_sums = [&](int nl, int n_slice) -> int {
        if (!sh) return I3D_OK;
        { TimedScope t(c, I3D_K_VECTOR); launch_lad_reduce_step(s, nl, part0.step, n_slice, red4, lv); }
        return allreduce(c, red4, (size_t)LADDER_MAX * 4);
    };
    int n_step = 0;
    set_slots();
    { TimedScope t(c, I3D_K_VECTOR); a.cur = st2; n_step = launch_pcg_step3_lad(s, 0 , B, a, lv); }
    for (int j = 0; j < B; ++j) finals[j] = st2 + 2 * j;
    const int seq0 = begin_passes(c);
    int it = 1;
    for (;; ++it) {
        set_slots();
        const int nl = (int)live.size();
        { const int rc = step_sums(nl, a.n_slice_wg); if (rc) return rc; }
        { TimedScope t(c, I3D_K_VECTOR);
          a.n_d2 = launch_pcg_dir3_lad(s, it == 1, nl, own, to, L.NS, Z0, P0, c->v_S.p, U0, ld.tail.p, c->v_cm.p, c->d_lm.p, part0.step, n_step, part0.d2, st2, (it + 1) & 1, c->d_flags, seq0 + it, lv,
                                       a.n_slice_wg, red4); }
        { const int n = rows_apply(it & 1, true); if (n < 0) return ctx_fail(c, I3D_ERR_STATE, "pcg_solve_ladder: the multi-system operator pass could not be launched"); a.n_pq = n; a.n_cam = n; }
        a.cur = st2 + (it & 1);
        if (it % PCG_RESET_PERIOD != 0) { TimedScope t(c, I3D_K_VECTOR); n_step = launch_pcg_step3_lad(s, 1, nl, a, lv); }
        else {
            { TimedScope t(c, I3D_K_VECTOR); launch_pcg_step3_lad(s, 2, nl, a, lv);
              for (int j : live) launch_u_from_x(c, L, X0 + (size_t)j * lv.vec, U0 + (size_t)j * lv.vec); }
            { const int n = rows_apply(it & 1, false); if (n < 0) return ctx_fail(c, I3D_ERR_STATE, "pcg_solve_ladder: the multi-system operator pass could not be launched"); a.n_cam = n; }
            { TimedScope t(c, I3D_K_VECTOR); n_step = launch_pcg_step3_lad(s, 3, nl, a, lv); }
        }
        {
            const int want = seq0 + it;
            std::vector<int> still;
            for (int j : live) {
                bool done = false;
                { const int rc = wait_pass(c, c->h_flags + 4 * j + 2 * (want & 1), want, "pcg_solve_ladder: the device stopped publishing its state", &done); if (rc) return rc; }
                if (!done) still.push_back(j);
                else finals[j] = st2 + 2 * j + (it & 1);
            }
            live.swap(still);
        }
        if (live.empty() || it > PCG_MAX_PASSES) break;
    }
    end_passes(c, seq0);
    for (int j : live) finals[j] = st2 + 2 * j + (it & 1);
    { const int lrc = ctx_launch_check(c); if (lrc) return lrc; }
    return I3D_OK;
}

}
```

### intrinsic3d_amd/csrc/host/solver.cpp

```cpp
#include "solver_internal.hpp"
#include <cstdlib>
#include <algorithm>

namespace i3d {

#ifdef I3D_MR_PHASES
void mr_phase_report_now();
#endif
#ifdef I3D_MR_BLOCKTIME
void mr_blocktime_report_now();
#endif

void read_switches(i3d_context* c) {
    auto env = [](const char* name) { return std::getenv(name); };
    auto is = [&](const char* name, char v) { const char* e = env(name); return e && e[0] == v; };
    auto num = [&](const char* name, int unset) { const char* e = env(name); return e ? std::atoi(e) : unset; };
    auto clamp = [](int v, int lo, int hi) { return v < lo ? lo : (v > hi ? hi : v); };
    SolverSwitches w;
    { const char* e = env("I3D_DETERMINISTIC"); w.deterministic = e ? (e[0] == '1' ? 1 : 0) : -1; }
    w.ladder = clamp(num("I3D_LADDER", LADDER_MAX), 1, LADDER_MAX);
    w.ladder_mr = !is("I3D_LADDER_MR", '0');
    w.ladder_mr1 = is("I3D_LADDER_MR1", '1');
    w.ladder_group = clamp(num("I3D_LADDER_GROUP", 3), 1, 3);
    w.ladder_pair = !is("I3D_LADDER_PAIR", '0');
    w.egt_mr1 = is("I3D_EGT_MR1", '1');
    { const char* e = env("I3D_EGT_TILE"); w.egt_tile = e ? (std::atoi(e) == 512 ? 512 : 1024) : 0; }
    w.hmax_limit = num("I3D_EGT_HMAX_LIMIT", 0);
    w.hmax_limit_1024 = num("I3D_EGT_HMAX_LIMIT_1024", 0);
    w.halo_pull = is("I3D_HALO_PULL", '1');
    w.no_tile = is("I3D_NO_TILE", '1');
    { const char* e = env("I3D_NO_CULL"); w.no_cull = (e && e[0] >= '1' && e[0] <= '3') ? e[0] - '0' : 0; }
    w.gradcol = !is("I3D_GRADCOL", '0');
    w.cost0 = !is("I3D_COST0", '0');
    w.debug_invalid_attempt = num("I3D_DEBUG_INVALID_ATTEMPT", -1);
    { const int v = num("I3D_SH_SLAB", 0); w.sh_slab = v > 0 ? v : 0; }
    c->sw = w;
}

static int wait_record(i3d_context* c, int idx, int seq, LmRecord& out) {
    LmRecord* const r = c->h_lmrec + idx;
    const double t0 = now_s();
    while (__atomic_load_n(&r->seq, __ATOMIC_ACQUIRE) != seq) {
        if (now_s() - t0 > 60.0) {
            CTX_HIP(c, sync_stream(c));
            if (__atomic_load_n(&r->seq, __ATOMIC_ACQUIRE) != seq) return ctx_fail(c, I3D_ERR_HIP, "lm_solve: the device stopped publishing the state of the trust-region loop");
        }
    }
    out = *r;
    return I3D_OK;
}

static SolveRoute solve_route(i3d_context* c) {
    const int NS = 6 * c->K + 9;
    const bool sh = c->sharded();
    SolveRoute rt; std::memset(&rt.reduce_dev, 0, sizeof(rt.reduce_dev));
    rt.multi_system = multi_system_ok(c);
    bool in_kernel = false;
    if (c->op.tile_ok && sh) { P2PDev probe; in_kernel = c->comm->fused_exchange(&probe) && NS + 2 <= probe.L.red_cap; }
    const bool three = c->op.tile_ok && (!sh || in_kernel);
    bool ladder = c->op.ladder_max > 1 && c->op.tile_ok && (sh ? !in_kernel : true) && rt.multi_system;
    if (ladder && alloc_ladder(c) != I3D_OK) {
        ladder = false;
    }
    rt.loop = ladder ? PcgLoop::Ladder : (three ? PcgLoop::ThreeLaunch : PcgLoop::SixLaunch);
    rt.exchange = !sh ? Exchange::None : (three ? Exchange::InKernel : Exchange::Transport);
    if (sh && rt.loop == PcgLoop::SixLaunch) {
        const bool ok = c->comm->device_reduce(&rt.reduce_dev) && NS + 1 <= rt.reduce_dev.L.red_cap;
        if (ok) rt.exchange = Exchange::InKernelReduce; else rt.reduce_dev.on = 0;
    }
    return rt;
}

static int lm_solve(i3d_context* c, const i3d_optimizer_config& cfg, OptParams& p, i3d_iteration_stats* st, double initial_radius) {
    hipStream_t s = c->stream;
    const Layout L = layout_of(c);
    const int N = c->N, K = c->K, NP = (int)L.NP, NS = L.NS;
    GridView g = c->grid_view(); RowView r = c->row_view();
    LadderState& ld = c->ladder;
    if (cfg.lm_steps > LM_REC_SLOTS - 2) return ctx_fail(c, I3D_ERR_CAPACITY, "optimize: more than 62 LM steps per outer iteration");
    const SolveRoute route = solve_route(c);
    { TimedScope t(c, I3D_K_VECTOR); launch_freemask(s, r, p, c->v_mask.p); }
    CTX_HIP(c, hipMemcpyAsync(c->xc_sdf.p, c->x_sdf.p, sizeof(double) * (size_t)N, hipMemcpyDeviceToDevice, s));
    CTX_HIP(c, hipMemcpyAsync(c->xc_alb.p, c->x_alb.p, sizeof(double) * (size_t)N, hipMemcpyDeviceToDevice, s));
    const bool one_stream = one_stream_gradcol(c);
    auto after_colnorm = [&]() -> int {
        CTX_HIP(c, hipMemcpyAsync(c->d_cam_c.p, c->d_shared.p, sizeof(double) * (size_t)NS, hipMemcpyDeviceToDevice, s));
        CTX_HIP(c, hipMemcpyAsync(c->d_cam_H.p, c->d_blocks.p, sizeof(double) * ((size_t)21 * K + 25), hipMemcpyDeviceToDevice, s));
        { int rc2 = allgather(c, c->v_c.p); if (rc2) return rc2; }
        { TimedScope t(c, I3D_K_VECTOR); launch_scale_from_colnorm(s, NP, c->v_c.p, c->v_mask.p, c->v_S.p, c->v_cm.p); }
        return I3D_OK;
    };
    int rc = I3D_OK;
    if (one_stream) { rc = run_gradcol(c, p, after_colnorm); if (rc) return rc; }
    else {
        rc = run_pass(c, PASS_COLNORM, p, nullptr, c->v_c.p); if (rc) return rc;
        rc = after_colnorm(); if (rc) return rc;
        rc = run_pass(c, PASS_GRAD, p, nullptr, c->v_acc.p); if (rc) return rc;
    }
    { TimedScope t(c, I3D_K_VECTOR); launch_mul(s, NP, c->v_S.p, c->v_acc.p, c->v_b.p); }
    if (!c->sw.cost0) { rc = eval_cost_launch(c, p, false, c->d_frames.p); if (rc) return rc; }
    else if (!one_stream) { TimedScope t(c, I3D_K_VECTOR); launch_set_double(s, c->d_scal.p + 16, c->cost_at_build); }
    rc = count_above_dev(c, c->v_acc.p, c->v_mask.p, 1e-10f, c->d_scal.p + 8); if (rc) return rc;
    rc = dot_dev(c, c->v_mask.p, c->v_mask.p, c->d_scal.p + 9); if (rc) return rc;
    {
        double* xs = c->h_pinned;
        for (int i = 0; i < 6 * K; ++i) xs[i] = c->poses[i];
        for (int i = 0; i < 4; ++i) xs[6 * K + i] = c->intr[i];
        for (int i = 0; i < 5; ++i) xs[6 * K + 4 + i] = c->dist[i];
        CTX_HIP(c, hipMemcpyAsync(c->d_xshared.p, xs, sizeof(double) * NS, hipMemcpyHostToDevice, s));
    }
    const int seq0 = c->lm_seq; c->lm_seq += LM_REC_SLOTS;
    LmState* const lm = c->d_lm.p;
    launch_lm_init(s, lm, c->d_scal.p + 16, c->d_scal.p + 8, c->d_scal.p + 9, initial_radius, c->d_lmrec, seq0);

    int attempts = 0; bool ended = false, accepted = false;
    auto consume = [&](const LmRecord& rec) {
        if (rec.kind == 0) {
            if (st) { st->cost_initial = rec.cost; st->cost_final = rec.cost; st->free_parameters = (int64_t)(rec.nfree + 0.5); st->termination = rec.final_ ? 1 : 0; st->final_radius = initial_radius; }
            c->last_sizes[5] = (long long)(rec.nfree + 0.5);
        } else if (rec.kind == 2) { if (st) st->termination = 1; }
        else {
            if (st) {
                st->lm_iterations = attempts + 1;
                if (attempts < 50) { st->pcg_iterations[attempts] = rec.pcg_it; st->step_accepted[attempts] = rec.accepted; }
                st->final_radius = rec.radius_after; st->termination = rec.termination;
                if (rec.accepted) { st->cost_final = rec.cost; st->successful_steps += 1; }
            }
            if (cfg.verbose) std::printf("  [i3d LM] it %d cand %.9e model %.3e rho %.4f radius -> %.3e cg %d%s\n", attempts + 1, rec.cand_cost, rec.model_change, rec.rel, rec.radius_after, rec.pcg_it,
                                         rec.accepted ? " accepted" : "");
            accepted = rec.accepted != 0;
            ++attempts;
        }
        if (rec.final_) ended = true;
    };
    auto queue_decision = [&](const float* x, const PcgState* ps, int attempt, int lad_next) -> int {
        { TimedScope t(c, I3D_K_VECTOR);
          launch_candidate(s, g, r, K, -1.0f, x, c->v_S.p, c->d_xshared.p, c->xc_sdf.p, c->xc_alb.p, c->d_xcshared.p, c->d_scal.p + 4, c->v_mask.p, c->d_partials.p, lm);
          launch_cand_frames(s, K, c->d_xcshared.p, c->d_frames.p, c->d_frames_cand.p, lm); }
        const int rc2 = eval_cost_launch(c, p, true, c->d_frames_cand.p, c->d_xcshared.p + 6 * K, lm); if (rc2) return rc2;
        { TimedScope t(c, I3D_K_VECTOR);
          launch_lm_decide(s, lm, ps, c->d_scal.p + 4, c->d_scal.p + 16, attempt, cfg.lm_steps, c->d_lmrec + 1 + attempt, seq0 + 1 + attempt, lad_next,
                           c->sw.debug_invalid_attempt == attempt ? 1 : 0);
          launch_accept(s, g, r, c->xc_sdf.p, c->xc_alb.p, lm); }
        return I3D_OK;
    };
    if (route.loop == PcgLoop::Ladder) {
        const LadVec& lv = ld.strides;
        { LmRecord rec; rc = wait_record(c, 0, seq0, rec); if (rc) return rc; consume(rec); }
        const bool warm = ld.hint > 0;
        int k = 0, prevB = 0; bool after_resync = false;
        while (k < cfg.lm_steps && !ended) {
            int B = after_resync ? 1 : (prevB == 0 ? (warm ? std::max(ld.hint, ld.hint_prev) : 2) : (warm ? 2 : 2 * prevB));
            B = std::max(1, std::min(B, std::min(c->op.ladder_max, cfg.lm_steps - k)));
            after_resync = false; prevB = B;
            { TimedScope t(c, I3D_K_VECTOR);
              launch_lm_begin_lad(s, lm, B, K, p.fix_poses, p.fix_intr, p.fix_dist, c->d_cam_c.p, c->d_cam_H.p, ld.mblk.p, lv.mblk, c->v_c.p + L.tail_off, c->v_S.p + L.tail_off, ld.tail.p, lv.tail,
                                  c->d_lmrec + 1 + k, seq0 + 1 + k); }
            const PcgState* fin[LADDER_MAX] = {nullptr};
            rc = pcg_solve_ladder(c, route, cfg, p, B, fin); if (rc) return rc;
            ++ld.batches;
            for (int j = 0; j < B && c->sharded(); ++j) { rc = allgather(c, lad_vecp(c, LV_X, j)); if (rc) return rc; }
            for (int j = 0; j < B; ++j) { rc = queue_decision(lad_vecp(c, LV_X, j), fin[j], k + j, j + 1); if (rc) return rc; }
            int decided = 0;
            for (int j = 0; j < B && !ended; ++j) {
                LmRecord rec; rc = wait_record(c, 1 + k + j, seq0 + 1 + k + j, rec); if (rc) return rc;
                if (rec.kind == 3) {
                    __atomic_store_n(&c->h_lmrec[1 + k + j].seq, 0, __ATOMIC_RELEASE);
                    ++ld.resyncs; after_resync = true; break;
                }
                consume(rec); ++decided;
            }
            if (ended && decided < B) ld.wasted += B - decided;
            k += decided;
        }
        if (attempts > 0) { ld.hint_prev = ld.hint; ld.hint = attempts; }
        ended = true;
    }
    const bool three = route.loop == PcgLoop::ThreeLaunch;
    int k = 0;
    for (; route.loop != PcgLoop::Ladder && k < cfg.lm_steps; ++k) {
        { TimedScope t(c, I3D_K_VECTOR);
          launch_lm_begin(s, lm, K, p.fix_poses, p.fix_intr, p.fix_dist, c->d_cam_c.p, c->d_cam_H.p, c->Minv_blocks.p, c->v_c.p + L.tail_off, c->v_S.p + L.tail_off, c->v_D2.p + L.tail_off, c->v_Minv.p + L.tail_off,
                          c->d_lmrec + 1 + k, seq0 + 1 + k);
          if (!three) launch_lm_diag_dev(s, (int)L.tail_off, c->v_c.p, c->v_S.p, lm, c->v_D2.p, c->v_Minv.p); }
        const PcgState* ps = nullptr;
        rc = three ? pcg_solve_fused(c, route, cfg, p, &ps) : pcg_solve(c, route, cfg, p, &ps); if (rc) return rc;
        { LmRecord rec; rc = wait_record(c, k, seq0 + k, rec); if (rc) return rc; consume(rec); }
        if (ended) break;
        { int rc2 = allgather(c, c->v_x.p); if (rc2) return rc2; }
        rc = queue_decision(c->v_x.p, ps, k, -1); if (rc) return rc;
    }
    if (!ended) { LmRecord rec; rc = wait_record(c, k, seq0 + k, rec); if (rc) return rc; consume(rec); }
    if (st) st->num_attempts = std::min(attempts, 50);
    CTX_HIP(c, hipMemcpyAsync(c->h_pinned, c->d_xcshared.p, sizeof(double) * NS, hipMemcpyDeviceToHost, s));
    CTX_HIP(c, sync_stream(c));
    if (c->sharded() && c->comm->health(s)) return ctx_fail(c, I3D_ERR_COMM, "lm_solve: a peer-to-peer exchange timed out (a rank stopped taking part)");
    if (accepted) {
        for (int i = 0; i < 6 * K; ++i) c->poses[i] = c->h_pinned[i];
        for (int i = 0; i < 4; ++i) c->intr[i] = c->h_pinned[6 * K + i];
        for (int i = 0; i < 5; ++i) c->dist[i] = c->h_pinned[6 * K + 4 + i];
    }
    { const int lrc = ctx_launch_check(c); if (lrc) return lrc; }
    return I3D_OK;
}

int optimize(i3d_context* c, const i3d_optimizer_config& cfg, i3d_iteration_stats* stats) {
    if (!c->have_grid || cfg.iterations < 1) return ctx_fail(c, I3D_ERR_INVALID_ARGUMENT, "optimize: no grid or iterations < 1");
    CTX_HIP(c, hipSetDevice(c->device));
    double carried_radius = 1e4;
    for (int itr = 0; itr < cfg.iterations; ++itr) {
        i3d_iteration_stats local; std::memset(&local, 0, sizeof(local));
        i3d_iteration_stats* st = stats ? &stats[itr] : &local;
        std::memset(st, 0, sizeof(*st));
        OptParams p;
        const double t0 = now_s();
        int rc = assemble(c, cfg, itr, p, st); if (rc) return rc;
        const double t1 = now_s();
        st->time_add = (c->t_add_end >= 0.0 && c->t_add_end <= t1 - t0) ? c->t_add_end : t1 - t0; st->time_build = (t1 - t0) - st->time_add;
        if (c->n_active > 0) { rc = lm_solve(c, cfg, p, st, cfg.carry_trust_radius ? carried_radius : 1e4); if (rc) return rc;
                               if (st->final_radius > 0.0) carried_radius = st->final_radius; }
        const double t2 = now_s();
        st->time_solve = t2 - t1;
        if (cfg.verbose) std::printf("[i3d] itr %d rows %lld/%lld/%lld/%lld valid %lld cost %.9e -> %.9e (add %.3f ms, solve %.3f ms)\n", itr,
                                     (long long)st->rows[0], (long long)st->rows[1], (long long)st->rows[2], (long long)st->rows[3], (long long)st->valid_voxels,
                                     st->cost_initial, st->cost_final, st->time_add * 1e3, st->time_solve * 1e3);
        timing_flush(c);
    }
    c->assembled = false;
#ifdef I3D_MR_PHASES
    mr_phase_report_now();
#endif
#ifdef I3D_MR_BLOCKTIME
    mr_blocktime_report_now();
#endif
    return I3D_OK;
}

}
```

Before: 43.96.

## Colocate ladder system workgroups, recompute z from r, and batch camera partial loads

The ladder PCG vector kernels now map a 1D grid so that workgroups of different systems interleave in groups of eight, with the tail workgroups scheduled first. The z vector is no longer stored in step3; instead dir3 recomputes z = Minv*r from the column norms, dropping one vector write and read per iteration. The camera-partial reduction loads eight values per thread before summing to raise memory-level parallelism, and step partials are written per workgroup index. These add recomputation in dir3 and a more complex block-to-work mapping, and they depend on bit-exact recomputation of z (contraction disabled) to keep results identical.

```diff
diff --git a/intrinsic3d_amd/csrc/device/kernels.hpp b/intrinsic3d_amd/csrc/device/kernels.hpp
--- a/intrinsic3d_amd/csrc/device/kernels.hpp
+++ b/intrinsic3d_amd/csrc/device/kernels.hpp
@@ -133,6 +133,11 @@
     size_t tail;
     int sysid[LADDER_MAX];
 };
+struct LadVecLayout {
+    bool colocate;
+    bool tail_first;
+    bool store_z;
+};
 struct Step3Args {
     int nq; int chunk4;
     const float4* p; const float4* qacc; float4* x; float4* r; const float4* b; float4* z;
@@ -159,10 +164,10 @@
 int  launch_pcg_step3(hipStream_t st, int mode , Step3Args a);
 void launch_halo_fold(hipStream_t st, RowView r, TilePlan t, float* qacc, const PcgState* state);
 void launch_pcg_init_lad(hipStream_t st, PcgState* st2_all , int B, int fixed_iterations, int max_iterations, const LmState* lm);
-int  launch_pcg_dir3_lad(hipStream_t st, bool init, int nsys, Seg2 sg, size_t tail_off, int ntail, const float* z0, float* p0, const float* S, float* u0, const float* tD2_0, const float* cm, const LmState* lm,
-                         const double* step_partials0, int n_step, double* d2_partials0, PcgState* st2_0, int prev_parity, int* host_flags0, int seq, const LadVec& lv,
-                         int n_slice_partials = 0, const double* red4_0 = nullptr );
-int  launch_pcg_step3_lad(hipStream_t st, int mode, int nsys, Step3Args a, const LadVec& lv);
+int  launch_pcg_dir3_lad(hipStream_t st, bool init, int nsys, Seg2 sg, size_t tail_off, int ntail, const float* z0, const float* r0, float* p0, const float* S, float* u0, const float* tD2_0, const float* cm,
+                         const LmState* lm, const double* step_partials0, int n_step, double* d2_partials0, PcgState* st2_0, int prev_parity, int* host_flags0, int seq, const LadVec& lv,
+                         const LadVecLayout& lay, int n_slice_partials = 0, const double* red4_0 = nullptr );
+int  launch_pcg_step3_lad(hipStream_t st, int mode, int nsys, Step3Args a, const LadVec& lv, const LadVecLayout& lay);
 void launch_lad_reduce_step(hipStream_t st, int nsys, const double* step_partials0, int n_slice, double* red4_0, const LadVec& lv);
 void launch_lad_reduce_op(hipStream_t st, int nsys, const float* cam_partials0, int n_cam, int cam_stride, int NS, const double* pq_partials0, int n_pq, const double* d2_partials0, int n_d2,
                           double* redop0, int redop_stride, const LadVec& lv);
diff --git a/intrinsic3d_amd/csrc/device/pcg_fused.hip b/intrinsic3d_amd/csrc/device/pcg_fused.hip
--- a/intrinsic3d_amd/csrc/device/pcg_fused.hip
+++ b/intrinsic3d_amd/csrc/device/pcg_fused.hip
@@ -47,8 +47,13 @@
 
 static __device__ inline void lm_from_colnorm(float cm, float inv_radius, float& s, float& d2, float& minv) { s = lm_scale(cm); lm_diag(cm, s, inv_radius, d2, minv); }
 
-template <int SH>
-static __device__ __forceinline__ void pcg_dir3_body(int init, int n4, int seg4, size_t tail_rel, int ntail, const float* __restrict__ z, float* __restrict__ p,
+static __device__ __forceinline__ float mul_rn(float a, float b) {
+#pragma clang fp contract(off)
+    return a * b;
+}
+
+template <int SH, bool ZR = false>
+static __device__ __forceinline__ void pcg_dir3_body(const int wg, const int nwg, int init, int n4, int seg4, size_t tail_rel, int ntail, const float* __restrict__ z, const float* __restrict__ r, float* __restrict__ p,
                                                         const float* __restrict__ S, float* __restrict__ u, const float* __restrict__ tD2 ,
                                                         const float* __restrict__ cm, const float inv_radius, const double* __restrict__ step_partials, int n_step, double* __restrict__ d2_partials,
                                                         const PcgState* __restrict__ prev, PcgState* __restrict__ next, int* host_flags, int seq, const ShardArgs& sa,
@@ -57,11 +62,11 @@
     __shared__ double smx[SH == 1 ? 4 * P2P_MAX_RANKS : 1];
     auto publish = [&](int done) { if (host_flags) { __hip_atomic_store(&host_flags[2 * (seq & 1) + 1], done, __ATOMIC_RELAXED, __HIP_MEMORY_SCOPE_SYSTEM);
                                                      __hip_atomic_store(&host_flags[2 * (seq & 1)], seq, __ATOMIC_RELEASE, __HIP_MEMORY_SCOPE_SYSTEM); } };
-    const int n_rim = SH == 1 ? sa.n_rim_wg : 0, n_main = SH ? (int)gridDim.x - n_rim - 1 : (int)gridDim.x;
-    const int lid = SH == 1 ? ((int)blockIdx.x < n_rim ? n_main + 1 + (int)blockIdx.x : (int)blockIdx.x - n_rim) : (int)blockIdx.x;
+    const int n_rim = SH == 1 ? sa.n_rim_wg : 0, n_main = SH ? nwg - n_rim - 1 : nwg;
+    const int lid = SH == 1 ? (wg < n_rim ? n_main + 1 + wg : wg - n_rim) : wg;
     const bool rim_wg = SH == 1 && lid > n_main, tail_wg = SH ? lid == n_main : lid == n_main - 1;
     const bool writer = lid == 0 && threadIdx.x == 0;
-    const float4* z4 = reinterpret_cast<const float4*>(z); float4* p4 = reinterpret_cast<float4*>(p);
+    const float4* z4 = reinterpret_cast<const float4*>(ZR ? r : z); float4* p4 = reinterpret_cast<float4*>(p);
     const float4* C4 = reinterpret_cast<const float4*>(cm); float4* u4 = reinterpret_cast<float4*>(u);
     if (prev->done) { if (writer) { *next = *prev; publish(prev->done); } return; }
     double tot[4];
@@ -136,11 +141,12 @@
         for (int j = lid * PF_THREADS + threadIdx.x; j < 2 * n4; j += n_main * PF_THREADS) {
             const int i = j < n4 ? j : j - n4 + seg4;
             float4 pi = z4[i]; const float4 cv = C4[i];
+            float4 sv, dd, mi;
+            lm_from_colnorm(cv.x, inv_radius, sv.x, dd.x, mi.x); lm_from_colnorm(cv.y, inv_radius, sv.y, dd.y, mi.y);
+            lm_from_colnorm(cv.z, inv_radius, sv.z, dd.z, mi.z); lm_from_colnorm(cv.w, inv_radius, sv.w, dd.w, mi.w);
+            if (ZR) { pi.x = mul_rn(mi.x, pi.x); pi.y = mul_rn(mi.y, pi.y); pi.z = mul_rn(mi.z, pi.z); pi.w = mul_rn(mi.w, pi.w); }
             if (!first) { const float4 po = p4[i]; pi.x += betaf * po.x; pi.y += betaf * po.y; pi.z += betaf * po.z; pi.w += betaf * po.w; }
             p4[i] = pi;
-            float4 sv, dd; float mi;
-            lm_from_colnorm(cv.x, inv_radius, sv.x, dd.x, mi); lm_from_colnorm(cv.y, inv_radius, sv.y, dd.y, mi);
-            lm_from_colnorm(cv.z, inv_radius, sv.z, dd.z, mi); lm_from_colnorm(cv.w, inv_radius, sv.w, dd.w, mi);
             u4[i] = make_float4(sv.x * pi.x, sv.y * pi.y, sv.z * pi.z, sv.w * pi.w);
             d2 += (double)dd.x * (double)pi.x * (double)pi.x + (double)dd.y * (double)pi.y * (double)pi.y + (double)dd.z * (double)pi.z * (double)pi.z + (double)dd.w * (double)pi.w * (double)pi.w;
         }
@@ -159,18 +165,32 @@
                                                         const float* __restrict__ S, float* __restrict__ u, const float* __restrict__ D2 ,
                                                         const float* __restrict__ cm, const LmState* __restrict__ lm, const double* __restrict__ step_partials, int n_step, double* __restrict__ d2_partials,
                                                         const PcgState* __restrict__ prev, PcgState* __restrict__ next, int* host_flags, int seq, ShardArgs sa) {
-    pcg_dir3_body<SH>(init, n4, seg4, tail_rel, ntail, z, p, S, u, D2 + tail_rel, cm, lm->inv_radius , step_partials, n_step, d2_partials, prev, next, host_flags, seq, sa);
-}
-template <bool COLL>
-__global__ void __launch_bounds__(PF_THREADS, 1) k_pcg_dir3_lad(int init, int n4, int seg4, size_t tail_rel, int ntail, const float* __restrict__ z0, float* __restrict__ p0,
+    pcg_dir3_body<SH>((int)blockIdx.x, (int)gridDim.x, init, n4, seg4, tail_rel, ntail, z, nullptr, p, S, u, D2 + tail_rel, cm, lm->inv_radius , step_partials, n_step, d2_partials, prev, next, host_flags, seq, sa);
+}
+struct LadWg { int slot, wg; };
+static __device__ __forceinline__ LadWg lad_wg(int nsys , int n_wg , int n_first ) {
+    if (nsys == 0) return LadWg{(int)blockIdx.y, (int)blockIdx.x};
+    int w = (int)blockIdx.x;
+    if (w < n_first * nsys) return LadWg{w % nsys, n_wg - n_first + w / nsys};
+    w -= n_first * nsys;
+    const int l = (w / (8 * nsys)) * 8 + (w & 7);
+    return LadWg{(w >> 3) % nsys, l < n_wg - n_first ? l : -1};
+}
+static int lad_grid(int nsys, int n_wg, int n_first) { return n_first * nsys + ((n_wg - n_first + 7) & ~7) * nsys; }
+
+template <bool COLL, bool ZR>
+__global__ void __launch_bounds__(PF_THREADS, 1) k_pcg_dir3_lad(int init, int n4, int seg4, size_t tail_rel, int ntail, const float* __restrict__ z0, const float* __restrict__ r0, float* __restrict__ p0,
                                                         const float* __restrict__ S, float* __restrict__ u0, const float* __restrict__ tD2_0, const float* __restrict__ cm, const LmState* __restrict__ lm,
                                                         const double* __restrict__ step_partials0, int n_step, double* __restrict__ d2_partials0, PcgState* __restrict__ st2_0 , int prev_parity,
-                                                        int* host_flags0, int seq, LadVec lv, int n_slice_partials, const double* __restrict__ red4_0) {
-    const int j = lv.sysid[blockIdx.y];
+                                                        int* host_flags0, int seq, LadVec lv, int n_slice_partials, const double* __restrict__ red4_0, int colo_nsys, int n_wg) {
+    const LadWg lw = lad_wg(COLL ? 0 : colo_nsys, n_wg, 0);
+    if (lw.wg < 0) return;
+    const int j = lv.sysid[lw.slot];
     ShardArgs none; none.n_rim_wg = 0; none.n_slice_partials = n_slice_partials;
     const size_t vo = (size_t)j * lv.vec;
-    pcg_dir3_body<COLL ? 2 : 0>(init, n4, seg4, tail_rel, ntail, z0 + vo, p0 + vo, S, u0 + vo, tD2_0 + (size_t)j * lv.tail, cm, lm->lad_inv_radius[j], step_partials0 + (size_t)j * lv.part, n_step,
-                                d2_partials0 + (size_t)j * lv.part, st2_0 + 2 * j + prev_parity, st2_0 + 2 * j + (prev_parity ^ 1), host_flags0 + 4 * j, seq, none, COLL ? red4_0 + 4 * j : nullptr);
+    pcg_dir3_body<COLL ? 2 : 0, ZR>(lw.wg, n_wg, init, n4, seg4, tail_rel, ntail, z0 + vo, ZR ? r0 + vo : nullptr, p0 + vo, S, u0 + vo, tD2_0 + (size_t)j * lv.tail, cm, lm->lad_inv_radius[j],
+                                    step_partials0 + (size_t)j * lv.part, n_step, d2_partials0 + (size_t)j * lv.part, st2_0 + 2 * j + prev_parity, st2_0 + 2 * j + (prev_parity ^ 1), host_flags0 + 4 * j, seq,
+                                    none, COLL ? red4_0 + 4 * j : nullptr);
 }
 
 static int dir3_main_wgs(int n_entries, int cap) { int b = (n_entries / 2 + PF_THREADS - 1) / PF_THREADS; b = b < 1 ? 1 : b; return b > cap ? cap : b; }
@@ -191,18 +211,25 @@
     return n_main;
 }
 
-int launch_pcg_dir3_lad(hipStream_t st, bool init, int nsys, Seg2 sg, size_t tail_off, int ntail, const float* z0, float* p0, const float* S, float* u0, const float* tD2_0, const float* cm, const LmState* lm,
-                        const double* step_partials0, int n_step, double* d2_partials0, PcgState* st2_0, int prev_parity, int* host_flags0, int seq, const LadVec& lv,
-                        int n_slice_partials, const double* red4_0) {
+int launch_pcg_dir3_lad(hipStream_t st, bool init, int nsys, Seg2 sg, size_t tail_off, int ntail, const float* z0, const float* r0, float* p0, const float* S, float* u0, const float* tD2_0, const float* cm,
+                        const LmState* lm, const double* step_partials0, int n_step, double* d2_partials0, PcgState* st2_0, int prev_parity, int* host_flags0, int seq, const LadVec& lv,
+                        const LadVecLayout& lay, int n_slice_partials, const double* red4_0) {
     const int n4 = sg.n >> 2, seg4 = (int)((sg.off1 - sg.off0) >> 2);
     const size_t o = sg.off0;
     const int blocks = dir3_main_wgs(sg.n, PF_MAX_WG);
-    if (red4_0)
-        k_pcg_dir3_lad<true><<<dim3(blocks + 1, nsys), PF_THREADS, 0, st>>>(init ? 1 : 0, n4, seg4, tail_off - o, ntail, z0 + o, p0 + o, S + o, u0 + o, tD2_0, cm + o, lm, step_partials0, n_step, d2_partials0,
-                                                                            st2_0, prev_parity, host_flags0, seq, lv, n_slice_partials, red4_0);
+    if (red4_0) {
+        k_pcg_dir3_lad<true, false><<<dim3(blocks + 1, nsys), PF_THREADS, 0, st>>>(init ? 1 : 0, n4, seg4, tail_off - o, ntail, z0 + o, nullptr, p0 + o, S + o, u0 + o, tD2_0, cm + o, lm, step_partials0, n_step,
+                                                                                   d2_partials0, st2_0, prev_parity, host_flags0, seq, lv, n_slice_partials, red4_0, 0, blocks + 1);
+        return blocks;
+    }
+    const dim3 grid = lay.colocate ? dim3(lad_grid(nsys, blocks, 0)) : dim3(blocks, nsys);
+    const int colo = lay.colocate ? nsys : 0;
+    if (lay.store_z || init)
+        k_pcg_dir3_lad<false, false><<<grid, PF_THREADS, 0, st>>>(init ? 1 : 0, n4, seg4, tail_off - o, ntail, z0 + o, nullptr, p0 + o, S + o, u0 + o, tD2_0, cm + o, lm, step_partials0, n_step, d2_partials0,
+                                                                  st2_0, prev_parity, host_flags0, seq, lv, 0, nullptr, colo, blocks);
     else
-        k_pcg_dir3_lad<false><<<dim3(blocks, nsys), PF_THREADS, 0, st>>>(init ? 1 : 0, n4, seg4, tail_off - o, ntail, z0 + o, p0 + o, S + o, u0 + o, tD2_0, cm + o, lm, step_partials0, n_step, d2_partials0,
-                                                                         st2_0, prev_parity, host_flags0, seq, lv, 0, nullptr);
+        k_pcg_dir3_lad<false, true><<<grid, PF_THREADS, 0, st>>>(init ? 1 : 0, n4, seg4, tail_off - o, ntail, z0 + o, r0 + o, p0 + o, S + o, u0 + o, tD2_0, cm + o, lm, step_partials0, n_step, d2_partials0,
+                                                                 st2_0, prev_parity, host_flags0, seq, lv, 0, nullptr, colo, blocks);
     return blocks;
 }
 
@@ -247,8 +274,8 @@
     }
 }
 
-template <int MODE, int SH>
-static __device__ __forceinline__ void pcg_step3_body(const Step3Args& a, const S3Off& o) {
+template <int MODE, int SH, bool STZ = true>
+static __device__ __forceinline__ void pcg_step3_body(const Step3Args& a, const S3Off& o, const int wg) {
     __shared__ double sm[4 * 8];
     __shared__ double smx[SH == 1 ? P2P_MAX_RANKS : 1];
     __shared__ double camv[64];
@@ -259,8 +286,8 @@
     const double* const pq_partials = a.pq_partials + o.part; const double* const d2_partials = a.d2_partials + o.part; double* const step_partials = a.step_partials + o.part;
     const float2* const qh = a.qh + o.qh2; const float* const cam_partials = a.cam_partials + o.cam; const float* const Mblk = a.Mblk + o.mblk;
     const float* const tp = a.tp + o.vo; float* const tx = a.tx + o.vo; float* const tr = a.tr + o.vo; float* const tz = a.tz + o.vo; const float* const tD2 = a.tD2 + o.tail;
-    const bool slice_wg = (int)blockIdx.x < a.n_slice_wg;
-    const int q0 = blockIdx.x * PF_THREADS + threadIdx.x, qstride = a.n_slice_wg * PF_THREADS;
+    const bool slice_wg = wg < a.n_slice_wg;
+    const int q0 = wg * PF_THREADS + threadIdx.x, qstride = a.n_slice_wg * PF_THREADS;
     S3In in;
     __shared__ int done_s;
     if (threadIdx.x == 0) done_s = cur->done;
@@ -274,14 +301,14 @@
         else reduce_partials_all<1>(pq_partials, a.n_pq, t1, sm, d2_partials, a.n_d2);
         if (SH == 1) {
             const unsigned e32 = p2p_pass_epoch(a.sh.seq, P2P_X_STEP);
-            if (blockIdx.x == 0 && threadIdx.x == 0) p2p_put_double_all(a.sh.pd, 1, e32, 0, t1[0]);
+            if (wg == 0 && threadIdx.x == 0) p2p_put_double_all(a.sh.pd, 1, e32, 0, t1[0]);
             p2p_sum_all<1>(a.sh.pd, 1, e32, t1, smx);
             t1[0] += d2_partials[a.n_d2];
         }
         const double pq = t1[0];
         const double al = cur->rho / pq;
         const bool bad = !(pq > 0.0) || isinf(pq) || isinf(al);
-        if (blockIdx.x == 0 && threadIdx.x == 0) { cur->pq = pq; if (bad) cur->done = 2; else cur->alpha = al; }
+        if (wg == 0 && threadIdx.x == 0) { cur->pq = pq; if (bad) cur->done = 2; else cur->alpha = al; }
         if (bad) return;
         alpha = (float)al;
     }
@@ -340,13 +367,13 @@
                     for (int k = 0; k < 4; ++k) { const double xd = xv[k]; s1 += xd * ((double)bv[k] + (double)rv[k]); s2 += xd * (double)rv[k]; s3 += (double)dv[k] * xd * xd; }
                 }
                 const float zv[4] = {mv[0] * rv[0], mv[1] * rv[1], mv[2] * rv[2], mv[3] * rv[3]};
-                Z[i] = make_float4(zv[0], zv[1], zv[2], zv[3]);
+                if (STZ) Z[i] = make_float4(zv[0], zv[1], zv[2], zv[3]);
 #pragma unroll
                 for (int k = 0; k < 4; ++k) s0 += (double)rv[k] * (double)zv[k];
             }
         }
     } else {
-        const int K = a.K, tw = (int)blockIdx.x - a.n_slice_wg, n_pose_wg = (K + PF_POSES_PER_WG - 1) / PF_POSES_PER_WG;
+        const int K = a.K, tw = wg - a.n_slice_wg, n_pose_wg = (K + PF_POSES_PER_WG - 1) / PF_POSES_PER_WG;
         int col0, ncol;
         if (tw < n_pose_wg) { col0 = 6 * PF_POSES_PER_WG * tw; const int c1 = min(6 * K, col0 + 6 * PF_POSES_PER_WG); ncol = c1 - col0; }
         else { col0 = 6 * K; ncol = 9; }
@@ -354,7 +381,17 @@
         if (MODE == S3_NORMAL || MODE == S3_RESET) {
             const int g = t / 64, c = t % 64;
             double v = 0.0;
-            if (SH != 2 && c < ncol) for (int w = g; w < a.n_cam; w += 8) v += (double)cam_partials[(size_t)w * a.cam_stride + col0 + c];
+            if (SH != 2 && c < ncol) {
+                const float* const cp = cam_partials + col0 + c;
+                for (int w0 = g; w0 < a.n_cam; w0 += 64) {
+                    float f[8];
+#pragma unroll
+                    for (int u = 0; u < 8; ++u) { const int w = w0 + 8 * u; f[u] = w < a.n_cam ? cp[(size_t)w * a.cam_stride] : 0.0f; }
+                    __builtin_amdgcn_sched_barrier(0);
+#pragma unroll
+                    for (int u = 0; u < 8; ++u) if (w0 + 8 * u < a.n_cam) v += (double)f[u];
+                }
+            }
             camred[g][c] = v;
             __syncthreads();
             if (t < ncol) {
@@ -402,15 +439,19 @@
         }
     }
     if (MODE == S3_XONLY) return;
-    block_partial_d(s0, step_partials, 4, 0); block_partial_d(s1, step_partials, 4, 1); block_partial_d(s2, step_partials, 4, 2); block_partial_d(s3, step_partials, 4, 3);
+    double* const mine = step_partials + 4 * (size_t)wg;
+    { const double t0 = block_sum_d(s0), t1 = block_sum_d(s1), t2 = block_sum_d(s2), t3 = block_sum_d(s3);
+      if (threadIdx.x == 0) { mine[0] = t0; mine[1] = t1; mine[2] = t2; mine[3] = t3; } }
 }
 template <int MODE, int SH>
-__global__ void __launch_bounds__(PF_THREADS) k_pcg_step3(Step3Args a) { const S3Off o{0, 0, 0, 0, 0, 0, 0, 0, -1}; pcg_step3_body<MODE, SH>(a, o); }
-template <int MODE, bool COLL>
-__global__ void __launch_bounds__(PF_THREADS) k_pcg_step3_lad(Step3Args a, LadVec lv) {
-    const int j = lv.sysid[blockIdx.y];
+__global__ void __launch_bounds__(PF_THREADS) k_pcg_step3(Step3Args a) { const S3Off o{0, 0, 0, 0, 0, 0, 0, 0, -1}; pcg_step3_body<MODE, SH>(a, o, (int)blockIdx.x); }
+template <int MODE, bool COLL, bool STZ>
+__global__ void __launch_bounds__(PF_THREADS) k_pcg_step3_lad(Step3Args a, LadVec lv, int colo_nsys, int n_wg, int n_first) {
+    const LadWg lw = lad_wg(COLL ? 0 : colo_nsys, n_wg, n_first);
+    if (lw.wg < 0) return;
+    const int j = lv.sysid[lw.slot];
     const S3Off o{((size_t)j * lv.vec) >> 2, (size_t)j * lv.vec, ((size_t)j * lv.qh) >> 1, (size_t)j * lv.part, (size_t)j * lv.cam, (size_t)j * lv.mblk, (size_t)j * lv.tail, 2 * j, j};
-    pcg_step3_body<MODE, COLL ? 2 : 0>(a, o);
+    pcg_step3_body<MODE, COLL ? 2 : 0, STZ>(a, o, lw.wg);
 }
 
 int pcg_step3_slice_wgs(int n_entries, int cap) { if (cap <= 0 || cap > PF_MAX_WG) cap = PF_MAX_WG; int b = (n_entries / 4 + PF_THREADS - 1) / PF_THREADS; return b < 1 ? 1 : (b > cap ? cap : b); }
@@ -429,10 +470,15 @@
     return mode == S3_XONLY ? 0 : blocks;
 }
 
-int launch_pcg_step3_lad(hipStream_t st, int mode, int nsys, Step3Args a, const LadVec& lv) {
-    const int blocks = a.n_slice_wg + pcg_step3_tail_wgs(a.K);
-    const dim3 grid(blocks, nsys);
-#define I3D_S3L(M) do { if (a.redop) k_pcg_step3_lad<M, true><<<grid, PF_THREADS, 0, st>>>(a, lv); else k_pcg_step3_lad<M, false><<<grid, PF_THREADS, 0, st>>>(a, lv); } while (0)
+int launch_pcg_step3_lad(hipStream_t st, int mode, int nsys, Step3Args a, const LadVec& lv, const LadVecLayout& lay) {
+    const int n_tail = pcg_step3_tail_wgs(a.K), blocks = a.n_slice_wg + n_tail;
+    const bool colo = lay.colocate && !a.redop;
+    const int n_first = colo && lay.tail_first ? n_tail : 0;
+    const dim3 grid = colo ? dim3(lad_grid(nsys, blocks, n_first)) : dim3(blocks, nsys);
+    const int cn = colo ? nsys : 0;
+#define I3D_S3L(M) do { if (a.redop) k_pcg_step3_lad<M, true, true><<<grid, PF_THREADS, 0, st>>>(a, lv, 0, blocks, 0); \
+                        else if (lay.store_z) k_pcg_step3_lad<M, false, true><<<grid, PF_THREADS, 0, st>>>(a, lv, cn, blocks, n_first); \
+                        else k_pcg_step3_lad<M, false, M == S3_INIT || M == S3_XONLY><<<grid, PF_THREADS, 0, st>>>(a, lv, cn, blocks, n_first); } while (0)
     switch (mode) {
         case S3_INIT:   I3D_S3L(S3_INIT); break;
         case S3_NORMAL: I3D_S3L(S3_NORMAL); break;
diff --git a/intrinsic3d_amd/csrc/host/context.hpp b/intrinsic3d_amd/csrc/host/context.hpp
--- a/intrinsic3d_amd/csrc/host/context.hpp
+++ b/intrinsic3d_amd/csrc/host/context.hpp
@@ -140,6 +140,7 @@
     int  deterministic = -1;
     int  ladder = LADDER_MAX;
     bool ladder_mr = true, ladder_mr1 = false, ladder_pair = true; int ladder_group = 3;
+    bool lad_vec_colocate = true, lad_tail_first = true, lad_store_z = false;
     bool egt_mr1 = false;
     int  egt_tile = 0;
     int  hmax_limit = 0, hmax_limit_1024 = 0;
diff --git a/intrinsic3d_amd/csrc/host/pcg.cpp b/intrinsic3d_amd/csrc/host/pcg.cpp
--- a/intrinsic3d_amd/csrc/host/pcg.cpp
+++ b/intrinsic3d_amd/csrc/host/pcg.cpp
@@ -305,6 +305,7 @@
     const int mr_cap = std::min(c->sw.ladder_group, eg_tile_mr_max_systems(K));
     const bool pair = c->sw.ladder_pair;
     const bool mr_ok = use_mr && mr_cap >= 1 && route.multi_system;
+    const LadVecLayout lay{c->sw.lad_vec_colocate, c->sw.lad_tail_first, c->sw.lad_store_z};
     const bool sh = route.exchange == Exchange::Transport;
     double* const red4 = sh ? ld.red.p : nullptr;
     const int rstride = (int)lad_redop_stride(L.NS);
@@ -360,7 +361,7 @@
     };
     int n_step = 0;
     set_slots();
-    { TimedScope t(c, I3D_K_VECTOR); a.cur = st2; n_step = launch_pcg_step3_lad(s, 0 , B, a, lv); }
+    { TimedScope t(c, I3D_K_VECTOR); a.cur = st2; n_step = launch_pcg_step3_lad(s, 0 , B, a, lv, lay); }
     for (int j = 0; j < B; ++j) finals[j] = st2 + 2 * j;
     const int seq0 = begin_passes(c);
     int it = 1;
@@ -369,16 +370,16 @@
         const int nl = (int)live.size();
         { const int rc = step_sums(nl, a.n_slice_wg); if (rc) return rc; }
         { TimedScope t(c, I3D_K_VECTOR);
-          a.n_d2 = launch_pcg_dir3_lad(s, it == 1, nl, own, to, L.NS, Z0, P0, c->v_S.p, U0, ld.tail.p, c->v_cm.p, c->d_lm.p, part0.step, n_step, part0.d2, st2, (it + 1) & 1, c->d_flags, seq0 + it, lv,
-                                       a.n_slice_wg, red4); }
+          a.n_d2 = launch_pcg_dir3_lad(s, it == 1, nl, own, to, L.NS, Z0, R0, P0, c->v_S.p, U0, ld.tail.p, c->v_cm.p, c->d_lm.p, part0.step, n_step, part0.d2, st2, (it + 1) & 1, c->d_flags, seq0 + it,
+                                       lv, lay, a.n_slice_wg, red4); }
         { const int n = rows_apply(it & 1, true); if (n < 0) return ctx_fail(c, I3D_ERR_STATE, "pcg_solve_ladder: the multi-system operator pass could not be launched"); a.n_pq = n; a.n_cam = n; }
         a.cur = st2 + (it & 1);
-        if (it % PCG_RESET_PERIOD != 0) { TimedScope t(c, I3D_K_VECTOR); n_step = launch_pcg_step3_lad(s, 1, nl, a, lv); }
+        if (it % PCG_RESET_PERIOD != 0) { TimedScope t(c, I3D_K_VECTOR); n_step = launch_pcg_step3_lad(s, 1, nl, a, lv, lay); }
         else {
-            { TimedScope t(c, I3D_K_VECTOR); launch_pcg_step3_lad(s, 2, nl, a, lv);
+            { TimedScope t(c, I3D_K_VECTOR); launch_pcg_step3_lad(s, 2, nl, a, lv, lay);
               for (int j : live) launch_u_from_x(c, L, X0 + (size_t)j * lv.vec, U0 + (size_t)j * lv.vec); }
             { const int n = rows_apply(it & 1, false); if (n < 0) return ctx_fail(c, I3D_ERR_STATE, "pcg_solve_ladder: the multi-system operator pass could not be launched"); a.n_cam = n; }
-            { TimedScope t(c, I3D_K_VECTOR); n_step = launch_pcg_step3_lad(s, 3, nl, a, lv); }
+            { TimedScope t(c, I3D_K_VECTOR); n_step = launch_pcg_step3_lad(s, 3, nl, a, lv, lay); }
         }
         {
             const int want = seq0 + it;
diff --git a/intrinsic3d_amd/csrc/host/solver.cpp b/intrinsic3d_amd/csrc/host/solver.cpp
--- a/intrinsic3d_amd/csrc/host/solver.cpp
+++ b/intrinsic3d_amd/csrc/host/solver.cpp
@@ -23,6 +23,9 @@
     w.ladder_mr1 = is("I3D_LADDER_MR1", '1');
     w.ladder_group = clamp(num("I3D_LADDER_GROUP", 3), 1, 3);
     w.ladder_pair = !is("I3D_LADDER_PAIR", '0');
+    w.lad_vec_colocate = !is("I3D_LAD_VEC_COLOCATE", '0');
+    w.lad_tail_first = !is("I3D_LAD_TAIL_FIRST", '0');
+    w.lad_store_z = is("I3D_LAD_STORE_Z", '1');
     w.egt_mr1 = is("I3D_EGT_MR1", '1');
     { const char* e = env("I3D_EGT_TILE"); w.egt_tile = e ? (std::atoi(e) == 512 ? 512 : 1024) : 0; }
     w.hmax_limit = num("I3D_EGT_HMAX_LIMIT", 0);
```

Result: faster. 44.97, median of 6 (+2.3%).
